# by256/icsg3d

Hardware: AMD Instinct MI355X
Metric: voxel-grids/s (fwd+bwd) for 32^3 U-Net+VAE at batch 32: value = U-Net train step (BASELINE configs[1]); DFC-VAE step (configs[2]) in secondary; both per batch in unet_plus_vae (higher is better)
Workload: dtype f32

## Files before the change

icsg3d_amd/csrc/common.h:

```cpp
#pragma once
#include <hip/hip_runtime.h>
#include <hip/hip_ext.h>
#include <atomic>
#include <cstdint>
#include <cstdio>
#include <string>
#include <vector>

namespace ics {

extern std::atomic<long long> g_kernel_launches;
struct LaunchTimer {
  virtual void next(hipEvent_t* start, hipEvent_t* stop) = 0;
  virtual ~LaunchTimer() = default;
};
extern thread_local LaunchTimer* tl_launch_timer;
template <typename... P, typename... A>
inline void ics_launch(void (*kernel)(P...), dim3 grid, dim3 block, size_t shmem, hipStream_t st, A&&... args) {
  static_assert(sizeof...(P) == sizeof...(A), "kernel argument count");
  if (tl_launch_timer != nullptr) {
    hipEvent_t e0 = nullptr, e1 = nullptr;
    tl_launch_timer->next(&e0, &e1);
    hipExtLaunchKernelGGL(kernel, grid, block, (std::uint32_t)shmem, st, e0, e1, 0u, static_cast<P>(args)...);
  } else {
    hipLaunchKernelGGL(kernel, grid, block, shmem, st, static_cast<P>(args)...);
  }
}
#define ICS_LAUNCH(...)                                      \
  do {                                                       \
    ::ics::g_kernel_launches.fetch_add(1, std::memory_order_relaxed); \
    ::ics::ics_launch(__VA_ARGS__);                          \
  } while (0)

void set_error(const std::string& msg);
#define ICS_HIP(expr)                                                                     \
  do {                                                                                    \
    hipError_t _e = (expr);                                                               \
    if (_e != hipSuccess) {                                                               \
      ::ics::set_error(std::string(#expr) + " -> " + hipGetErrorString(_e) + " @" +       \
                       __FILE__ + ":" + std::to_string(__LINE__));                        \
      return -1;                                                                          \
    }                                                                                     \
  } while (0)
#define ICS_CHECK(cond, msg)                                                              \
  do {                                                                                    \
    if (!(cond)) {                                                                        \
      ::ics::set_error(std::string(msg) + " (" #cond ") @" + __FILE__ + ":" +             \
                       std::to_string(__LINE__));                                         \
      return -1;                                                                          \
    }                                                                                     \
  } while (0)
#define ICS_TRY(expr)                                                                     \
  do {                                                                                    \
    if ((expr) != 0) return -1;                                                           \
  } while (0)

enum Act : int { ACT_NONE = 0, ACT_RELU = 1, ACT_LRELU = 2 };
constexpr float kLeaky = 0.3f;
constexpr float kBnEps = 1e-3f;
constexpr float kKEps = 1e-7f;
constexpr float kPoolTieTol = 1e-5f;

__device__ __forceinline__ float act_fwd(float v, int act) {
  if (act == ACT_RELU) return fmaxf(v, 0.f);
  if (act == ACT_LRELU) return v > 0.f ? v : kLeaky * v;
  return v;
}
__device__ __forceinline__ float act_grad(float v, int act) {
  if (act == ACT_RELU) return v > 0.f ? 1.f : 0.f;
  if (act == ACT_LRELU) return v > 0.f ? 1.f : kLeaky;
  return 1.f;
}

struct ConvSrc {
  const float* p;
  const float* scale;
  const float* shift;
  int C;
  int up;
  int act;
  int bcast;
};

enum ConvFlags : int {
  CF_NO_REUSE = 1,
  CF_NO_WGRAD3 = 2,
  CF_NO_WGRAD3S = 4,
  CF_NO_FWD_SPLITK = 8,
  CF_NO_THIN_N = 16,
  CF_NO_UPSPLIT = 32,
  CF_NO_THIN_C = 64,
  CF_NO_COND_FOLD = 128,
  CF_NO_WINO = 256,
  CF_NO_WINO_WGRAD = 512,
  CF_NO_WINO64 = 1024,
  CF_NO_UP3 = 2048,
  CF_NO_THIN1_2STAGE = 4096,
  CF_NO_FAST_BNBWD = 8192,
  CF_NO_FUSED_HEAD = 16384,
  CF_NO_BWD_FOLD = 32768,
  CF_UP3_BIG_ALWAYS = 65536,
  CF_NO_WINOG = 262144,
  CF_NO_HEAD_BNFUSE = 524288,
  CF_NO_UP3N = 1 << 21,
  CF_NO_DGRAD_BNFUSE = 1 << 22,
  CF_NO_POOL_PRESUM = 1 << 23,
  CF_NO_HEAD_LABELS = 1 << 24,
  CF_ZBATCH = 1 << 20,
};
int conv_flags_from_env();

struct ConvGeom {
  int B, S, lgS;
  int Cin, Cout;
  int taps;
  int Kpad, Npad;
  int flags = 0;
};

struct BwdStat {
  const float* s = nullptr;
  const float* mean = nullptr;
  const float* rstd = nullptr;
  const float* scale = nullptr;
  const float* shift = nullptr;
  float* partial = nullptr;
  int post_act = ACT_NONE;
  int ld = 0;
  const float* abc = nullptr;
  float* db_partial = nullptr;
  const float* pool_d = nullptr;
  int pool_ld = 0;
  const unsigned char* pool_mask = nullptr;
};

int launch_conv_fwd(hipStream_t st, const ConvGeom& g, const ConvSrc* src, int nsrc,
                    const float* wpacked, const float* bias, float* out, int ldo, int pre_act,
                    float* stat_partial, int* stat_rows_per_block, int accumulate = 0,
                    float* splitk_ws = nullptr, size_t splitk_ws_floats = 0, const BwdStat* bwd = nullptr,
                    int* bwd_blocks = nullptr);
size_t conv_fwd_workspace_floats(const ConvGeom& g, const ConvSrc* src, int nsrc);
bool conv_thin_c_ok(const ConvGeom& g, const ConvSrc& s0, int nsrc, int cin_log);
size_t conv_thin_c_wgrad_workspace_floats(const ConvGeom& g);
int launch_conv_wgrad_thin_c(hipStream_t st, const ConvGeom& g, const ConvSrc& s0, const float* dy, int ldy, float* dw,
                             int ldw, int row_pitch, float* ws, size_t ws_floats, int phase);
int launch_conv_fwd_thin_c(hipStream_t st, const ConvGeom& g, const ConvSrc& s0, int cin_log, int wstride,
                           const float* wp, const float* bias, float* out, int ldo, int pre_act, float* stat_partial,
                           int* rows_per_block, const float* pos_bias = nullptr);
int launch_conv_fwd_par(hipStream_t st, const ConvGeom& g_lowres, const ConvSrc& src, const float* wpar, float* out,
                        int ldo, const float* bias = nullptr, int pre_act = ACT_NONE, float* stat_partial = nullptr,
                        int* stat_blocks = nullptr);
int launch_pack_par(hipStream_t st, const float* w, int Cin_total, int Cout, int c_off, int Cu, float* dst, int Kpad,
                    int Npad);
int launch_pack_fwd_sub(hipStream_t st, const float* w, int taps, int Cin_total, int Cout, int c_off, int Csub,
                        float* dst, int Kpad, int Npad);
int launch_conv_wgrad(hipStream_t st, const ConvGeom& g, const ConvSrc* src, int nsrc,
                      const float* dy, int ldy, float* dw, int ldw, float* workspace,
                      size_t workspace_floats, int sub_rows = 0, int row_pitch = 0, int row_off = 0,
                      int phase = 0);
const char* conv_last_kernel_id();
void conv_set_last_kernel_id(const char* id);
int launch_pack_sub(hipStream_t st, const float* w, int taps, int Cin_total, int Cout, int c_off, int Csub,
                    int flip, float* dst, int Kpad, int Npad);
size_t conv_wgrad_workspace_floats(const ConvGeom& g, const ConvSrc* src, int nsrc);
int conv_fwd_rows_per_block(const ConvGeom& g);
int launch_conv_wgrad_ablate(hipStream_t st, const ConvGeom& g, const ConvSrc* src, const float* dy, int ldy,
                             float* workspace, int ablate);
int launch_conv_fwd_ablate(hipStream_t st, const ConvGeom& g, const ConvSrc* src, int nsrc, const float* wp,
                           float* out, int ldo, int ablate);
int launch_pack_fwd(hipStream_t st, const float* w, int K, int N, float* dst, int Kpad, int Npad,
                    int k_off, int n_off, int zero_first, int cin_log = 0, int cin_phys = 0);
void* pack_table_record_begin();
int pack_table_record_end(void* handle, std::vector<unsigned char>* bytes, int* njobs, unsigned* nblocks);
int launch_pack_table(hipStream_t st, const void* d_jobs, int njobs, unsigned nblocks);
int launch_materialize_input(hipStream_t st, const ConvSrc* src, int nsrc, int Cin, int CinG, int B, int S,
                             float* out);
int launch_pack_bwd(hipStream_t st, const float* w, int taps, int Cin, int Cout, float* dst,
                    int Kpad, int Npad, int cout_total, int co_off, int zero_first);

bool conv_wino_ok(const ConvGeom& g, const ConvSrc* src, int nsrc);
size_t conv_wino_weight_floats(int Cin, int Cout);
int launch_conv_fwd_wino(hipStream_t st, const ConvGeom& g, const ConvSrc& s0, const float* wt, const float* bias,
                         float* out, int ldo, int pre_act, float* stat_partial, int* rows_per_block, int accumulate,
                         int layout, const BwdStat* bwd = nullptr, int* bwd_blocks = nullptr);
int launch_pack_wino(hipStream_t st, const float* w, int Cin_total, int Cout, int c_off, int Csub, int bwd, float* dst,
                     int layout = 0);
int conv_wino_layout(const ConvGeom& g);
bool conv_wino64_ok(const ConvGeom& g, const ConvSrc* src, int nsrc);
int launch_conv_fwd_wino64(hipStream_t st, const ConvGeom& g, const ConvSrc& s0, const float* wt, const float* bias,
                           float* out, int ldo, int pre_act, float* stat_partial, int* rows_per_block, int accumulate,
                           const BwdStat* bwd = nullptr, int* bwd_blocks = nullptr);
bool conv_wino_wgrad_ok(const ConvGeom& g, const ConvSrc* src, int nsrc);
size_t conv_wino_wgrad_workspace_floats(const ConvGeom& g);
int launch_conv_wgrad_wino(hipStream_t st, const ConvGeom& g, const ConvSrc& s0, const float* dy, int ldy, float* dw,
// ... 26 lines not shown
```

icsg3d_amd/csrc/conv_igemm.hip:

```cpp
#include "common.h"

#ifndef ICS_GEMM_DEEP_FWD_MIN
#define ICS_GEMM_DEEP_FWD_MIN 1
#endif
#ifndef ICS_GEMM_DEEP_MIN
#define ICS_GEMM_DEEP_MIN 3
#endif
#ifndef ICS_GEMM_DEEP
#define ICS_GEMM_DEEP 1
#endif

#include <algorithm>
#include <type_traits>
#include <cstdlib>
#include <cstring>
#include <vector>

namespace ics {

typedef float f32x16 __attribute__((ext_vector_type(16)));
typedef float v4f __attribute__((ext_vector_type(4)));

#ifndef ICS_KLDA
#define ICS_KLDA 36
#endif
constexpr int kLDA = ICS_KLDA;

__device__ __forceinline__ int xcd_swizzle(int bid, int nblk) {
  const int xcd = bid & 7, q = nblk >> 3, r = nblk & 7;
  return (xcd < r ? xcd * (q + 1) : r * (q + 1) + (xcd - r) * q) + (bid >> 3);
}

static thread_local const char* g_last_kernel_id = "";
const char* conv_last_kernel_id() { return g_last_kernel_id; }
void conv_set_last_kernel_id(const char* id) { g_last_kernel_id = id; }
static const char* tf(bool b) { return b ? "true" : "false"; }

int conv_flags_from_env() {
  int f = 0;
  if (getenv("ICSG3D_NO_REUSE")) f |= CF_NO_REUSE;
  if (getenv("ICSG3D_NO_WGRAD3")) f |= CF_NO_WGRAD3;
  if (getenv("ICSG3D_NO_WGRAD3S")) f |= CF_NO_WGRAD3S;
  if (getenv("ICSG3D_NO_FWD_SPLITK")) f |= CF_NO_FWD_SPLITK;
  if (getenv("ICSG3D_NO_THIN_N")) f |= CF_NO_THIN_N;
  if (getenv("ICSG3D_NO_UPSPLIT")) f |= CF_NO_UPSPLIT;
  if (getenv("ICSG3D_NO_THIN_C")) f |= CF_NO_THIN_C;
  if (getenv("ICSG3D_NO_COND_FOLD")) f |= CF_NO_COND_FOLD;
  if (getenv("ICSG3D_NO_WINO")) f |= CF_NO_WINO;
  if (getenv("ICSG3D_NO_WINO_WGRAD")) f |= CF_NO_WINO_WGRAD;
  if (getenv("ICSG3D_NO_WINO64")) f |= CF_NO_WINO64;
  if (getenv("ICSG3D_NO_UP3")) f |= CF_NO_UP3;
  if (getenv("ICSG3D_NO_THIN1_2STAGE")) f |= CF_NO_THIN1_2STAGE;
  if (getenv("ICSG3D_NO_FAST_BNBWD")) f |= CF_NO_FAST_BNBWD;
  if (getenv("ICSG3D_NO_FUSED_HEAD")) f |= CF_NO_FUSED_HEAD;
  if (getenv("ICSG3D_NO_BWD_FOLD")) f |= CF_NO_BWD_FOLD;
  if (getenv("ICSG3D_NO_WINOG")) f |= CF_NO_WINOG;
  if (getenv("ICSG3D_NO_HEAD_BNFUSE")) f |= CF_NO_HEAD_BNFUSE;
  if (getenv("ICSG3D_NO_UP3N")) f |= CF_NO_UP3N;
  if (getenv("ICSG3D_NO_DGRAD_BNFUSE")) f |= CF_NO_DGRAD_BNFUSE;
  if (getenv("ICSG3D_NO_POOL_PRESUM")) f |= CF_NO_POOL_PRESUM;
  if (getenv("ICSG3D_NO_HEAD_LABELS")) f |= CF_NO_HEAD_LABELS;
  { const char* e = getenv("ICSG3D_UP3_BIG_MIN_WG"); if (e && *e && strtoul(e, nullptr, 10) <= 1) f |= CF_UP3_BIG_ALWAYS; }
  return f;
}
struct DevOnce {
  bool done[64] = {false};
  bool need(int* dev) {
    int d = 0;
    if (hipGetDevice(&d) != hipSuccess || d < 0 || d >= 64) { *dev = -1; return true; }
    *dev = d;
    return !done[d];
  }
  void mark(int dev) { if (dev >= 0) done[dev] = true; }
};

static int identity_affine(const float** ones, const float** zeros) {
  constexpr int kN = 16384;
  static float* buf[64] = {nullptr};
  int dev = 0;
  ICS_HIP(hipGetDevice(&dev));
  ICS_CHECK(dev >= 0 && dev < 64, "device index out of range");
  if (!buf[dev]) {
    float* p = nullptr;
    ICS_HIP(hipMalloc(&p, 2 * kN * sizeof(float)));
    std::vector<float> h(2 * kN, 0.f);
    for (int i = 0; i < kN; ++i) h[i] = 1.f;
    ICS_HIP(hipMemcpy(p, h.data(), 2 * kN * sizeof(float), hipMemcpyHostToDevice));
    buf[dev] = p;
  }
  *ones = buf[dev];
  *zeros = buf[dev] + kN;
  return 0;
}
static int fix_src(ConvSrc& s) {
  if (s.scale == nullptr) {
    ICS_CHECK(s.C <= 16384, "source wider than the identity-affine buffer");
    ICS_TRY(identity_affine(&s.scale, &s.shift));
    s.act = ACT_NONE;
  }
  return 0;
}

struct RowPos {
  int b, z, y, x;
};
__device__ __forceinline__ RowPos decode_row(int m, int S, int lg) {
  RowPos r;
  r.x = m & (S - 1);
  r.y = (m >> lg) & (S - 1);
  r.z = (m >> (2 * lg)) & (S - 1);
  r.b = m >> (3 * lg);
  return r;
}

// ... 10 lines not shown
}
__device__ __forceinline__ float act_apply(float v, float slope) {
  return fmaxf(v, v * slope);
}
template <bool NOACT>
__device__ __forceinline__ v4f affine_only_or_act4(v4f v, v4f sc, v4f sh, float slope);
__device__ __forceinline__ v4f affine_act4(v4f v, v4f sc, v4f sh, float slope) {
  v4f r;
  r.x = act_apply(fmaf(v.x, sc.x, sh.x), slope); r.y = act_apply(fmaf(v.y, sc.y, sh.y), slope);
  r.z = act_apply(fmaf(v.z, sc.z, sh.z), slope); r.w = act_apply(fmaf(v.w, sc.w, sh.w), slope);
  return r;
}
template <bool NOACT>
__device__ __forceinline__ v4f affine_only_or_act4(v4f v, v4f sc, v4f sh, float slope) {
  if (!NOACT) return affine_act4(v, sc, sh, slope);
  v4f r;
  r.x = fmaf(v.x, sc.x, sh.x); r.y = fmaf(v.y, sc.y, sh.y); r.z = fmaf(v.z, sc.z, sh.z); r.w = fmaf(v.w, sc.w, sh.w);
  return r;
}
__device__ __forceinline__ unsigned voxel_off(int b, int z, int y, int x, int S, int u, int C) {
  const int Ss = S >> u;
  return ((((unsigned)b * Ss + (z >> u)) * Ss + (y >> u)) * Ss + (x >> u)) * (unsigned)C;
}
__device__ __forceinline__ int clampi(int v, int hi) { return min(max(v, 0), hi); }

__device__ __forceinline__ ConvSrc pick_src(const ConvSrc& s0, const ConvSrc& s1, bool first) {
  ConvSrc s;
  s.p = first ? s0.p : s1.p;
  s.scale = first ? s0.scale : s1.scale;
  s.shift = first ? s0.shift : s1.shift;
  s.C = first ? s0.C : s1.C;
  s.up = first ? s0.up : s1.up;
  s.act = first ? s0.act : s1.act;
  s.bcast = first ? s0.bcast : s1.bcast;
  return s;
}

__device__ __forceinline__ float gather_scalar(const ConvSrc& s0, const ConvSrc& s1, int ci, int b,
                                               int z, int y, int x, int S) {
  const bool first = ci < s0.C;
  const ConvSrc s = pick_src(s0, s1, first);
  const int cl = first ? ci : ci - s0.C;
  float v;
  if (s.bcast > 0) {
    v = s.p[(size_t)b * s.bcast + (cl % s.bcast)];
  } else {
    v = s.p[src_voxel(s, b, z, y, x, S) + cl];
  }
  if (s.scale) v = act_fwd(fmaf(v, s.scale[cl], s.shift[cl]), s.act);
  return v;
}

template <int WM, int WN, int TM, int TN, bool VEC, int ABL = 0, bool AFF = true, bool UP = true, bool THIN = false,
          bool REUSE = false, bool PAR = false, bool NOACT = false, bool FOLD = false>
__global__ __launch_bounds__(256, FOLD ? 2 : ((REUSE && PAR) ? 3 : 1)) void conv_fwd_kernel(ConvGeom g, ConvSrc s0, ConvSrc s1,
                                                        const float* __restrict__ wp,
                                                        const float* __restrict__ bias,
                                                        float* __restrict__ out, int ldo, int pre_act,
                                                        float* __restrict__ stat_partial, int gridM,
                                                        int gridN, int accumulate, BwdStat bs) {
  constexpr int BM = WM * TM * 32, BN = WN * TN * 32;
  constexpr int B_FLOATS = 32 * BN;
  constexpr int RA = BM / 32;
  constexpr int RS = BM / 8;
  constexpr int NB = BN / 32;
  extern __shared__ __attribute__((aligned(16))) float smem[];
  const int A_FLOATS = (REUSE ? BM + (BM >> g.lgS) + 1 : BM) * kLDA;
  float* As = smem;
  constexpr int NABUF = 1;
  float* Bs = smem + NABUF * A_FLOATS;

  const int t = threadIdx.x, lane = t & 63, wave = t >> 6;
  const int wm = wave / WN, wn = wave % WN;
  const int li = lane & 31, lh = lane >> 5;
  const int sw = xcd_swizzle(blockIdx.x, gridM * gridN);
  const int mb = sw / gridN, nb = sw % gridN;
  const int S = g.S, lg = g.lgS;
  const int M = g.B << (3 * lg);
  const int n0 = nb * BN;
  const int nchunks = g.Kpad >> 5;
  const int cpt = (VEC && !THIN) ? (g.Cin >> 5) : 1;
  const int cls = PAR ? (int)blockIdx.y : 0;
  const int pz = cls >> 2, py = (cls >> 1) & 1, px = cls & 1;
  if (PAR) wp += (size_t)cls * g.Kpad * g.Npad;
  const bool zbatch = (g.flags & CF_ZBATCH) != 0;
  if (zbatch) {
    s0.p += (size_t)blockIdx.z * (size_t)M * (size_t)s0.C;
    wp += (size_t)blockIdx.z * (size_t)g.Kpad * (size_t)g.Npad;
    out += (size_t)blockIdx.z * (size_t)M * (size_t)ldo;
  }
  const int zsplit = zbatch ? 1 : (int)gridDim.z, zidx = zbatch ? 0 : (int)blockIdx.z;

  const int mrow_base = mb * BM + (VEC ? (t >> 3) : (t >> 5));
  const float slope0 = act_slope_of(s0.act), slope1 = act_slope_of(s1.act);
  const float pre_slope = act_slope_of(pre_act);

  unsigned rmask[RA];
  int rvh[RA];
  if (VEC) {
#pragma unroll
    for (int r = 0; r < RA; ++r) {
      const int m = mrow_base + 32 * r;
      const RowPos rp = decode_row(m, S, lg);
      unsigned mk = 0;
      if (m < M) {
        if (PAR) {
#pragma unroll
          for (int tp = 0; tp < 8; ++tp) {
            const int zz = rp.z + (tp >> 2) + pz - 1, yy = rp.y + ((tp >> 1) & 1) + py - 1, xx = rp.x + (tp & 1) + px - 1;
            const bool ok = (unsigned)zz < (unsigned)S && (unsigned)yy < (unsigned)S && (unsigned)xx < (unsigned)S;
            mk |= (ok ? 1u : 0u) << tp;
          }
#pragma unroll
// ... 118 lines not shown
#pragma unroll
      for (int r = 0; r < RA; ++r) {
        const unsigned mk = rmask[r];
        const bool inb = kvalid && ((mk >> (tap & 31)) & 1u);
        int idx = mrow_base + 32 * r + sdelta;
        if (UP) {
          const int ez = (dz + (int)((mk >> 29) & 1u)) >> 1;
          const int ey = (dy + (int)((mk >> 28) & 1u)) >> 1;
          const int ex = (dx + (int)((mk >> 27) & 1u)) >> 1;
          const int idx_up = rvh[r] + (ez * Sh + ey) * Sh + ex;
          idx = su ? idx_up : idx;
        }
        const unsigned off = inb ? (unsigned)idx * (unsigned)sC + cl : (unsigned)cl;
        if (ABL == 3) {
          ra4[r] = *reinterpret_cast<const v4f*>(sp + (((unsigned)(mrow_base + 32 * r) * sC + c * 32 + cl) & 0xffffffu));
          continue;
        }
        if (ABL == 8) {
          ra4[r] = *reinterpret_cast<const v4f*>(sp + ((unsigned)max(idx, 0) * (unsigned)sC + cl));
          continue;
        }
        if (ABL == 9) {
          const v4f vv = *reinterpret_cast<const v4f*>(sp + (((unsigned)(mrow_base + 32 * r) * sC + c * 32 + cl) & 0xffffffu));
          ra4[r] = inb ? vv : v4f{0.f, 0.f, 0.f, 0.f};
          continue;
        }
        v4f v = *reinterpret_cast<const v4f*>(sp + off);
        if (AFF && ABL != 4) v = affine_act4(v, sc, sh, slope);
        ra4[r] = inb ? v : v4f{0.f, 0.f, 0.f, 0.f};
      }
    } else {
      const int kf = (c << 5) + (t & 31);
      const int tap = kf / g.Cin, ci = kf - tap * g.Cin;
      const bool kvalid = tap < g.taps;
      int dz = 0, dy = 0, dx = 0;
      if (g.taps == 27) { dz = tap / 9 - 1; dy = (tap / 3) % 3 - 1; dx = tap % 3 - 1; }
#pragma unroll
      for (int r = 0; r < RS; ++r) {
        const int m = mrow_base + 8 * r;
        const RowPos rp = decode_row(m, S, lg);
        const int zz = rp.z + dz, yy = rp.y + dy, xx = rp.x + dx;
        const bool inb = kvalid && m < M && (unsigned)zz < (unsigned)S &&
                         (unsigned)yy < (unsigned)S && (unsigned)xx < (unsigned)S;
        ras[r] = inb ? gather_scalar(s0, s1, ci, rp.b, zz, yy, xx, S) : 0.f;
      }
    }
  };

  unsigned rowG0[RA], rowG1[RA];
  if (VEC) {
#pragma unroll
    for (int r = 0; r < RA; ++r) {
      const unsigned mc = (unsigned)min(mrow_base + 32 * r, M - 1);
      rowG0[r] = (mc * (unsigned)s0.C + (unsigned)(t & 7) * 4u) * 4u;
      rowG1[r] = (mc * (unsigned)s1.C + (unsigned)(t & 7) * 4u) * 4u;
    }
  }
  auto load_chunk_gemm = [&](int c) {
    load_b(c * 8);
    const int ci0 = c << 5;
    const bool first = ci0 < s0.C;
    const int cbase = first ? ci0 : ci0 - s0.C;
    const char* sp = reinterpret_cast<const char*>(first ? s0.p : s1.p) + (size_t)cbase * 4;
    const float slope = first ? slope0 : slope1;
    v4f sc = v4f{1.f, 1.f, 1.f, 1.f}, sh = v4f{0.f, 0.f, 0.f, 0.f};
    if (AFF) {
      sc = *reinterpret_cast<const v4f*>((first ? s0.scale : s1.scale) + cbase + (t & 7) * 4);
      sh = *reinterpret_cast<const v4f*>((first ? s0.shift : s1.shift) + cbase + (t & 7) * 4);
    }
#pragma unroll
    for (int r = 0; r < RA; ++r) {
      v4f v = *reinterpret_cast<const v4f*>(sp + (first ? rowG0[r] : rowG1[r]));
      if (AFF) v = affine_only_or_act4<NOACT>(v, sc, sh, slope);
      ra4[r] = v;
    }
  };
  auto store_a_chunk = [&]() {
    float* A = As;
    if (VEC) {
#pragma unroll
      for (int r = 0; r < RA; ++r)
        *reinterpret_cast<v4f*>(A + ((t >> 3) + 32 * r) * kLDA + (t & 7) * 4) = ra4[r];
    } else {
#pragma unroll
      for (int r = 0; r < RS; ++r) A[((t >> 5) + 8 * r) * kLDA + (t & 31)] = ras[r];
    }
  };

  f32x16 acc[TM][TN];
#pragma unroll
  for (int i = 0; i < TM; ++i)
#pragma unroll
    for (int j = 0; j < TN; ++j)
#pragma unroll
      for (int r = 0; r < 16; ++r) acc[i][j][r] = 0.f;
  if (accumulate && !PAR && zsplit == 1) {
#pragma unroll
    for (int j = 0; j < TN; ++j) {
      const int n = n0 + wn * TN * 32 + j * 32 + li;
#pragma unroll
      for (int i = 0; i < TM; ++i)
#pragma unroll
        for (int r = 0; r < 16; ++r) {
          const int m = mb * BM + wm * TM * 32 + 4 * lh + i * 32 + (r & 3) + 8 * (r >> 2);
          if (m < M && n < g.Cout) acc[i][j][r] = out[(size_t)m * ldo + n];
        }
    }
  }

  auto compute_at = [&](const float* Abase, int arow_stride_rows, int bbuf) {
    const float* Bw = Bs + bbuf * B_FLOATS + (lh * BN + wn * TN * 32 + li) * 4;
#pragma unroll
    for (int g8 = 0; g8 < 4; ++g8) {
      float4 a[TM], b[TN];
#pragma unroll
      for (int i = 0; i < TM; ++i)
// ... 73 lines not shown
    store_b(par);
    __syncthreads();
    for (int G = G0; G + 1 < G1; ++G) {
      int ngzy = gzy, ncc = cc + 1;
      if (ncc == cpt) { ncc = 0; ++ngzy; }
      load_a_group(ngzy, ncc);
#pragma unroll
      for (int i = 0; i < NDX; ++i) {
        load_b(i + 1 < NDX ? b_rows(gzy, cc, i + 1) : b_rows(ngzy, ncc, 0));
        compute_reuse(0, par, dx_first + i);
        par ^= 1;
        store_b(par);
        __syncthreads();
      }
      store_a_group(0);
      __syncthreads();
      gzy = ngzy; cc = ncc;
    }
    {
#pragma unroll
      for (int i = 0; i + 1 < NDX; ++i) {
        load_b(b_rows(gzy, cc, i + 1));
        compute_reuse(0, par, dx_first + i);
        par ^= 1;
        store_b(par);
        __syncthreads();
      }
      compute_reuse(0, par, dx_first + NDX - 1);
      __syncthreads();
    }
    }
  } else {
  int cb = 0, ce = nchunks;
  if (zsplit > 1) {
    const int per = (nchunks + zsplit - 1) / zsplit;
    cb = zidx * per;
    ce = min(nchunks, cb + per);
  }
  const bool gemm = VEC && !THIN && !PAR && !UP && ABL == 0 && g.taps == 1;
  if (cb < ce && gemm) {
    auto compute_g = [&](int buf) { compute_at(As + (wm * TM * 32 + li) * kLDA + lh * 4, 32, buf); };
    load_chunk_gemm(cb);
    store_b(cb & 1);
    store_a_chunk();
    __syncthreads();
#if ICS_GEMM_DEEP
    if (!AFF && TM * TN >= ICS_GEMM_DEEP_FWD_MIN) {
      v4f raA[RA], rbA[NB], raB[RA], rbB[NB];
      auto load_set = [&](int c, v4f (&xa)[RA], v4f (&xb)[NB]) {
        const char* wrow = reinterpret_cast<const char*>(wp) + (size_t)(c * 8) * (size_t)g.Npad * 16;
#pragma unroll
        for (int r = 0; r < NB; ++r) xb[r] = *reinterpret_cast<const v4f*>(wrow + bofs[r]);
        const int ci0 = c << 5;
        const bool first = ci0 < s0.C;
        const char* sp = reinterpret_cast<const char*>(first ? s0.p : s1.p) + (size_t)(first ? ci0 : ci0 - s0.C) * 4;
#pragma unroll
        for (int r = 0; r < RA; ++r) xa[r] = *reinterpret_cast<const v4f*>(sp + (first ? rowG0[r] : rowG1[r]));
      };
      auto store_set = [&](int buf, const v4f (&xa)[RA], const v4f (&xb)[NB]) {
        float* Bw = Bs + buf * B_FLOATS;
#pragma unroll
        for (int r = 0; r < NB; ++r) *reinterpret_cast<v4f*>(Bw + (t + 256 * r) * 4) = xb[r];
        __syncthreads();
#pragma unroll
        for (int r = 0; r < RA; ++r) *reinterpret_cast<v4f*>(As + ((t >> 3) + 32 * r) * kLDA + (t & 7) * 4) = xa[r];
        __syncthreads();
      };
      const int lastc = ce - 1;
      if (cb + 1 < ce) load_set(cb + 1, raA, rbA);
      int c = cb;
      for (; c + 2 < ce; c += 2) {
        load_set(c + 2, raB, rbB);
        compute_g(c & 1);
        store_set((c + 1) & 1, raA, rbA);
        load_set(c + 3 < ce ? c + 3 : lastc, raA, rbA);
        compute_g((c + 1) & 1);
        store_set(c & 1, raB, rbB);
      }
      if (c + 1 < ce) {
        compute_g(c & 1);
        store_set((c + 1) & 1, raA, rbA);
      }
      compute_g((ce - 1) & 1);
      __syncthreads();
    } else
#endif
    {
    for (int c = cb; c + 1 < ce; ++c) {
      load_chunk_gemm(c + 1);
      compute_g(c & 1);
      store_b((c + 1) & 1);
      __syncthreads();
      store_a_chunk();
      __syncthreads();
    }
    compute_g((ce - 1) & 1);
    __syncthreads();
    }
  } else if (cb < ce) {
  load_chunk(cb);
  store_b(cb & 1);
  store_a_chunk();
  __syncthreads();

  auto compute = [&](int buf) {
    compute_at(As + (wm * TM * 32 + li) * kLDA + lh * 4, 32, buf);
  };
  auto compute_regs_only = [&]() {
// ... 111 lines not shown
  }
  if (stat_partial == nullptr) return;

  float* red = smem;
  float* bmean = smem + WM * BN;
  const int nvalid_rows = min(BM, M - mb * BM);
#pragma unroll
  for (int j = 0; j < TN; ++j) {
    float cs = colsum[j];
    cs += __shfl_xor(cs, 32);
    if (lh == 0) red[wm * BN + wn * TN * 32 + j * 32 + li] = cs;
  }
  __syncthreads();
  if (t < BN) {
    float s = 0.f;
#pragma unroll
    for (int w = 0; w < WM; ++w) s += red[w * BN + t];
    bmean[t] = s / (float)nvalid_rows;
  }
  __syncthreads();
#pragma unroll
  for (int j = 0; j < TN; ++j) {
    const float mu = bmean[wn * TN * 32 + j * 32 + li];
    float q = 0.f;
#pragma unroll
    for (int i = 0; i < TM; ++i)
#pragma unroll
      for (int r = 0; r < 16; ++r) {
        const int m = mrow0 + i * 32 + (r & 3) + 8 * (r >> 2);
        const float d = acc[i][j][r] - mu;
        q += (m < M) ? d * d : 0.f;
      }
    q += __shfl_xor(q, 32);
    colsum[j] = q;
  }
  __syncthreads();
#pragma unroll
  for (int j = 0; j < TN; ++j)
    if (lh == 0) red[wm * BN + wn * TN * 32 + j * 32 + li] = colsum[j];
  __syncthreads();
  if (t < BN) {
    float q = 0.f;
#pragma unroll
    for (int w = 0; w < WM; ++w) q += red[w * BN + t];
    const size_t nstat = (size_t)(PAR ? 8 : 1) * gridM;
    float* sp = stat_partial + (size_t)(n0 + t) * nstat + (size_t)(cls * gridM + mb);
    sp[0] = (float)nvalid_rows;
    sp[(size_t)g.Npad * nstat] = bmean[t];
    sp[(size_t)2 * g.Npad * nstat] = q;
  }
}

template <int WM, int WN, int TM, int TN, bool VEC, int ABL = 0, bool AFF = true, bool UP = true, bool THIN = false,
          bool REUSE = false, bool PAR = false, bool NOACT = false, bool FOLD = false>
static int launch_fwd_cfg(hipStream_t st, const ConvGeom& g, const ConvSrc& s0, const ConvSrc& s1,
                          const float* wp, const float* bias, float* out, int ldo, int pre_act,
                          float* stat_partial, int* rows_per_block, int accumulate = 0, int ksplit = 1,
                          const BwdStat* bwd = nullptr) {
  constexpr int BM = WM * TM * 32, BN = WN * TN * 32;
  const int M = g.B << (3 * g.lgS);
  const int gridM = (M + BM - 1) / BM, gridN = g.Npad / BN;
  const int arows = REUSE ? BM + (BM >> g.lgS) + 1 : BM;
  const size_t lds = (size_t)(arows * kLDA + 2 * 32 * BN) * sizeof(float);
  auto kern = conv_fwd_kernel<WM, WN, TM, TN, VEC, ABL, AFF, UP, THIN, REUSE, PAR, NOACT, FOLD>;
  static DevOnce attr;
  int dev;
  if (attr.need(&dev)) {
    const size_t lds_max = (size_t)((REUSE ? BM + BM / 4 + 1 : BM) * kLDA + 2 * 32 * BN) * sizeof(float);
    ICS_HIP(hipFuncSetAttribute(reinterpret_cast<const void*>(kern),
                                hipFuncAttributeMaxDynamicSharedMemorySize, (int)lds_max));
    attr.mark(dev);
  }
  if (rows_per_block) *rows_per_block = BM;
  static const std::string id = std::string("conv_fwd_kernel<") + std::to_string(WM) + ", " + std::to_string(WN) + ", " +
                                std::to_string(TM) + ", " + std::to_string(TN) + ", " + tf(VEC) + ", " +
                                std::to_string(ABL) + ", " + tf(AFF) + ", " + tf(UP) + ", " + tf(THIN) + ", " +
                                tf(REUSE) + ", " + tf(PAR) + ", " + tf(NOACT) + ", " + tf(FOLD) + ">";
  g_last_kernel_id = id.c_str();
  BwdStat bs_arg;
  if (FOLD) bs_arg = *bwd;
  ICS_LAUNCH(kern, dim3(gridM * gridN, PAR ? 8 : 1, ksplit), dim3(256), lds, st, g, s0, s1, wp, bias, out, ldo,
                     pre_act, stat_partial, gridM, gridN, accumulate, bs_arg);
  ICS_HIP(hipGetLastError());
  return 0;
}

static void pick_fwd_tile(const ConvGeom& g, int* bm, int* bn) {
  const int M = g.B << (3 * g.lgS);
  int BN = (g.Npad % 128 == 0) ? 128 : (g.Npad % 96 == 0) ? 96 : (g.Npad % 64 == 0) ? 64 : 32;
  int BM = 128;
  if (g.Npad % 64 == 0 && (long)((M + 127) / 128) * (g.Npad / BN) < 384) {
    BM = 64;
    BN = 64;
  }
  *bm = BM;
  *bn = BN;
}

static bool fwd_is_vec(const ConvGeom& g, const ConvSrc& s0, const ConvSrc& s1) {
  return (g.Cin % 32 == 0) && (s0.C % 32 == 0) && s0.bcast == 0 && s1.bcast == 0;
}
static bool conv_is_thin(const ConvGeom& g, const ConvSrc& s0, int nsrc) {
  return nsrc == 1 && s0.bcast == 0 && s0.C == g.Cin && (g.Cin == 4 || g.Cin == 8 || g.Cin == 16);
}


int launch_gemm_zbatch(hipStream_t st, int nz, int M, int K, int N, const float* A, const float* Wp, float* out, int flags) {
  ICS_CHECK(nz >= 1 && nz <= 65535 && M >= 1 && K % 32 == 0 && N % 64 == 0, "z-batched GEMM: K % 32, N % 64 required");
  ICS_CHECK((size_t)M * (size_t)std::max(K, N) < ((size_t)1 << 30), "z-batched GEMM: matrix too large for 32-bit offsets");
  const ConvGeom g{M, 1, 0, K, N, 1, K, N, flags | CF_ZBATCH};
  const ConvSrc s0{A, nullptr, nullptr, K, 0, ACT_NONE, 0}, s1{};
#ifndef ICS_ZB_BIG
#define ICS_ZB_BIG 1
#endif
  if (ICS_ZB_BIG && M % 128 == 0 && N % 128 == 0 && (long)(M / 128) * (N / 128) * nz >= 512)
    return launch_fwd_cfg<2, 2, 2, 2, true, 0, false, false, false, false, false, true, false>(
        st, g, s0, s1, Wp, nullptr, out, N, ACT_NONE, nullptr, nullptr, 0, nz);
  return launch_fwd_cfg<2, 2, 1, 1, true, 0, false, false, false, false, false, true, false>(
      st, g, s0, s1, Wp, nullptr, out, N, ACT_NONE, nullptr, nullptr, 0, nz);
}

int conv_fwd_rows_per_block(const ConvGeom& g) {
  int bm, bn;
  pick_fwd_tile(g, &bm, &bn);
  if (g.taps == 27 && g.Cout <= 4 && g.Cin % 4 == 0 && g.Cin >= 4 && g.Cin <= 64) {
    bm = std::min(bm, g.Cin <= 16 ? 256 : 64);
  }
  return bm;
}

#ifndef ICS_THINC_UNROLL
#define ICS_THINC_UNROLL 3
#endif
template <int CIN, int COUT>
__global__ __launch_bounds__(256) void conv_thin_c_fwd_kernel(ConvGeom g, const float* __restrict__ x, int wstride,
                                                               const float* __restrict__ wp,
                                                               const float* __restrict__ bias,
                                                               float* __restrict__ out, int ldo, int pre_act,
                                                               float* __restrict__ stat_partial,
                                                               const float* __restrict__ pos_bias) {
  constexpr int LPV = COUT / 4;
  constexpr int GPB = 256 / LPV;
  constexpr int VPB = 4 * GPB;
  constexpr int C4 = CIN >= 4 ? CIN / 4 : 1;
  extern __shared__ __attribute__((aligned(16))) float smem[];
  float* w = smem;
  const int t = threadIdx.x;
  const int S = g.S, lg = g.lgS;
  const int M = g.B << (3 * lg);
// ... 734 lines not shown
  if (ks > 1 && (size_t)ks * ((size_t)g.B << (3 * g.lgS)) * g.Npad > ws_floats) ks = 1;
  if (bwd_blocks) *bwd_blocks = 0;
  if (ks <= 1) {
    const bool fold = bwd != nullptr && bwd->partial != nullptr && !thin_n_ok(g, src[0], nsrc) &&
                      fwd_is_vec(g, s0, s1) && !conv_is_thin(g, s0, nsrc) && s0.scale == nullptr && !s0.up &&
                      (nsrc < 2 || (s1.scale == nullptr && !s1.up)) && bias == nullptr && stat_partial == nullptr &&
                      !accumulate;
    int rpb = 0;
    ICS_TRY(launch_conv_fwd_inner(st, g, src, nsrc, wp, bias, out, ldo, pre_act, stat_partial, &rpb, accumulate, 1,
                                  fold ? bwd : nullptr, ws, ws_floats));
    if (rows_per_block) *rows_per_block = rpb;
    if (fold && bwd_blocks) *bwd_blocks = (int)((((size_t)g.B << (3 * g.lgS)) + rpb - 1) / rpb);
    return 0;
  }
  const int M = g.B << (3 * g.lgS);
  ICS_CHECK((size_t)ks * M * g.Npad <= ws_floats, "forward split-K workspace too small");
  ICS_TRY(launch_conv_fwd_inner(st, g, src, nsrc, wp, nullptr, ws, g.Npad, ACT_NONE, nullptr, nullptr, 0, ks));
  ICS_LAUNCH(splitk_finish_kernel, dim3((M + 63) / 64, (g.Npad + 63) / 64), dim3(256), 0, st, ws, ks, M, g.Cout,
                     g.Npad, bias, act_slope_of(pre_act), out, ldo, accumulate, stat_partial);
  ICS_HIP(hipGetLastError());
  if (rows_per_block) *rows_per_block = 64;
  return 0;
}

static int launch_conv_fwd_inner(hipStream_t st, const ConvGeom& g, const ConvSrc* src, int nsrc,
                                 const float* wp, const float* bias, float* out, int ldo, int pre_act,
                                 float* stat_partial, int* rows_per_block, int accumulate, int ksplit,
                                 const BwdStat* bwd, float* ws, size_t ws_floats) {
  if (ksplit == 1 && thin_n_ok(g, src[0], nsrc))
    return launch_thin_n_fwd(st, g, src[0], wp, bias, out, ldo, pre_act, stat_partial, rows_per_block, accumulate, ws,
                             ws_floats);
  if (ksplit == 1 && !accumulate && bwd == nullptr && conv_thin_c_ok(g, src[0], nsrc, g.Cin) && ldo % 4 == 0)
    return launch_conv_fwd_thin_c(st, g, src[0], g.Cin, g.Cin, wp, bias, out, ldo, pre_act, stat_partial,
                                  rows_per_block);
  ConvSrc s0 = src[0], s1 = src[nsrc > 1 ? 1 : 0];
  if (nsrc == 1) s1.C = 0;
  const bool aff = s0.scale != nullptr || (nsrc > 1 && s1.scale != nullptr);
  const bool up = s0.up || (nsrc > 1 && s1.up);
  const int variant = up ? 2 : (aff ? 1 : 0);
  const bool noact = aff && (s0.scale == nullptr || s0.act == ACT_NONE) &&
                     (nsrc < 2 || s1.scale == nullptr || s1.act == ACT_NONE);
  ICS_TRY(fix_src(s0));
  ICS_TRY(fix_src(s1));
  bool vec = fwd_is_vec(g, s0, s1);
  const bool thin = conv_is_thin(g, s0, nsrc);
  ICS_CHECK(((size_t)g.B << (3 * g.lgS)) * (size_t)std::max(s0.C, s1.C) * 4 <= 0xffffffffull,
            "conv source larger than 4 GiB");
  const bool no_reuse = (g.flags & CF_NO_REUSE) != 0;
  const bool fold = bwd != nullptr && bwd->partial != nullptr && ksplit == 1 && vec && !thin && variant == 0 &&
                    bias == nullptr && stat_partial == nullptr && !accumulate;
  int bm, bn;
  pick_fwd_tile(g, &bm, &bn);
#define ICS_FWD_ARGS st, g, s0, s1, wp, bias, out, ldo, pre_act, stat_partial, rows_per_block, accumulate, ksplit, bwd
#define ICS_FWD(WM, WN, TM, TN)                                                                 \
  do {                                                                                          \
    if (thin) return launch_fwd_cfg<WM, WN, TM, TN, true, 0, true, true, true>(ICS_FWD_ARGS);   \
    if (!vec) return launch_fwd_cfg<WM, WN, TM, TN, false, 0, true, true>(ICS_FWD_ARGS);        \
    if (g.taps == 27 && g.S >= 4 && g.S <= (WM) * (TM) * 32 && !no_reuse) {                      \
      if (variant == 0 && fold)                                                                 \
        return launch_fwd_cfg<WM, WN, TM, TN, true, 0, false, false, false, true, false, false, true>(ICS_FWD_ARGS); \
      if (variant == 0) return launch_fwd_cfg<WM, WN, TM, TN, true, 0, false, false, false, true>(ICS_FWD_ARGS); \
      if (variant == 1 && noact)                                                                \
        return launch_fwd_cfg<WM, WN, TM, TN, true, 0, true, false, false, true, false, true>(ICS_FWD_ARGS);     \
      if (variant == 1) return launch_fwd_cfg<WM, WN, TM, TN, true, 0, true, false, false, true>(ICS_FWD_ARGS);  \
      return launch_fwd_cfg<WM, WN, TM, TN, true, 0, true, true, false, true>(ICS_FWD_ARGS);    \
    }                                                                                           \
    if (variant == 0 && fold)                                                                   \
      return launch_fwd_cfg<WM, WN, TM, TN, true, 0, false, false, false, false, false, false, true>(ICS_FWD_ARGS); \
    if (variant == 0) return launch_fwd_cfg<WM, WN, TM, TN, true, 0, false, false>(ICS_FWD_ARGS); \
    if (variant == 1) return launch_fwd_cfg<WM, WN, TM, TN, true, 0, true, false>(ICS_FWD_ARGS);  \
    return launch_fwd_cfg<WM, WN, TM, TN, true, 0, true, true>(ICS_FWD_ARGS);                   \
  } while (0)
  if (bm == 64) { ICS_FWD(2, 2, 1, 1); }
  if (bn == 128) { ICS_FWD(2, 2, 2, 2); }
  if (bn == 96) { ICS_FWD(4, 1, 1, 3); }
  if (bn == 64) { ICS_FWD(2, 2, 2, 1); }
  ICS_FWD(4, 1, 1, 1);
#undef ICS_FWD_ARGS
#undef ICS_FWD
}

static void pick_par_tile(const ConvGeom& g, int* bm, int* bn) {
  pick_fwd_tile(g, bm, bn);
  if (*bm == 64 && g.Npad % 128 == 0 && (long)(((g.B << (3 * g.lgS)) + 127) / 128) * (g.Npad / 128) * 8 >= 384) {
    *bm = 128; *bn = 128;
  }
}
int launch_conv_fwd_par(hipStream_t st, const ConvGeom& g, const ConvSrc& src, const float* wp, float* out,
                        int ldo, const float* bias, int pre_act, float* stat_partial, int* stat_blocks) {
  ConvSrc s0 = src, s1 = src;
  s1.C = 0;
  ICS_CHECK(g.taps == 8 && g.Cin % 32 == 0 && s0.C == g.Cin && !s0.up && !s0.bcast && g.Kpad == 8 * g.Cin,
            "parity-class conv needs a direct 32k-channel source");
  ICS_TRY(fix_src(s0));
  ICS_TRY(fix_src(s1));
  int bm, bn;
  pick_par_tile(g, &bm, &bn);
  int rpb = 0;
#define ICS_PAR_ARGS st, g, s0, s1, wp, bias, out, ldo, pre_act, stat_partial, &rpb
  int rc;
  const bool no_reuse = (g.flags & CF_NO_REUSE) != 0;
  const bool reuse = !no_reuse && g.S >= 4 && g.S <= bm;
  const bool noact = src.scale != nullptr && src.act == ACT_NONE;
#define ICS_PAR(WM, WN, TM, TN)                                                                              \
  (reuse ? (noact ? launch_fwd_cfg<WM, WN, TM, TN, true, 0, true, false, false, true, true, true>(ICS_PAR_ARGS) \
                  : launch_fwd_cfg<WM, WN, TM, TN, true, 0, true, false, false, true, true>(ICS_PAR_ARGS))   \
// ... 58 lines not shown
  const size_t total = (size_t)8 * Kpad * Npad;
  ICS_LAUNCH(pack_par_kernel, dim3((unsigned)((total + 255) / 256)), dim3(256), 0, st, w, Cin_total, Cout,
                     c_off, Cu, dst, Kpad, Npad);
  ICS_HIP(hipGetLastError());
  return 0;
}
__device__ __forceinline__ float pack_fwd_sub_value(size_t i, const float* __restrict__ w, int taps, int Cin_total,
                                                    int Cout, int c_off, int Csub, int Npad) {
  const int tq = i & 3;
  const size_t rest = i >> 2;
  const int n = rest % Npad;
  const int k = (int)(rest / Npad) * 4 + tq;
  const int tap = k / Csub, c = k - tap * Csub;
  return (tap < taps && n < Cout) ? w[((size_t)tap * Cin_total + c_off + c) * Cout + n] : 0.f;
}
__global__ void pack_fwd_sub_kernel(const float* __restrict__ w, int taps, int Cin_total, int Cout, int c_off,
                                    int Csub, float* __restrict__ dst, int Kpad, int Npad) {
  const size_t i = (size_t)blockIdx.x * blockDim.x + threadIdx.x;
  if (i >= (size_t)Kpad * Npad) return;
  dst[i] = pack_fwd_sub_value(i, w, taps, Cin_total, Cout, c_off, Csub, Npad);
}
int launch_pack_fwd_sub(hipStream_t st, const float* w, int taps, int Cin_total, int Cout, int c_off, int Csub,
                        float* dst, int Kpad, int Npad) {
  if (g_pack_rec) { g_pack_rec->push_back(PackJob{3, w, dst, {taps, Cin_total, Cout, c_off, Csub, Npad, 0, 0, 0}, (unsigned long long)Kpad * Npad, 0}); return 0; }
  const size_t total = (size_t)Kpad * Npad;
  ICS_LAUNCH(pack_fwd_sub_kernel, dim3((unsigned)((total + 255) / 256)), dim3(256), 0, st, w, taps,
                     Cin_total, Cout, c_off, Csub, dst, Kpad, Npad);
  ICS_HIP(hipGetLastError());
  return 0;
}

int launch_conv_fwd_ablate(hipStream_t st, const ConvGeom& g, const ConvSrc* src, int nsrc, const float* wp,
                           float* out, int ldo, int ablate) {
  ConvSrc s0 = src[0], s1 = src[nsrc > 1 ? 1 : 0];
  if (nsrc == 1) s1.C = 0;
  ICS_TRY(fix_src(s0));
  ICS_TRY(fix_src(s1));
  ICS_CHECK(fwd_is_vec(g, s0, s1) && g.Npad % 128 == 0, "ablation bench needs the vector 128x128 configuration");
#define ICS_ABL_ARGS st, g, s0, s1, wp, nullptr, out, ldo, 0, nullptr, nullptr
  if (ablate == 1) return launch_fwd_cfg<2, 2, 2, 2, true, 1, true, false>(ICS_ABL_ARGS);
  if (ablate == 2) return launch_fwd_cfg<2, 2, 2, 2, true, 2, true, false>(ICS_ABL_ARGS);
  if (ablate == 3) return launch_fwd_cfg<2, 2, 2, 2, true, 3, true, false>(ICS_ABL_ARGS);
  if (ablate == 4) return launch_fwd_cfg<2, 2, 2, 2, true, 4, true, false>(ICS_ABL_ARGS);
  if (ablate == 8) return launch_fwd_cfg<2, 2, 2, 2, true, 8, false, false>(ICS_ABL_ARGS);
  if (ablate == 9) return launch_fwd_cfg<2, 2, 2, 2, true, 9, false, false>(ICS_ABL_ARGS);
  if (ablate == 5) return launch_fwd_cfg<2, 2, 2, 2, true, 0, true, false>(ICS_ABL_ARGS);
  if (ablate == 6) return launch_fwd_cfg<2, 2, 2, 2, true, 0, true, true>(ICS_ABL_ARGS);
  return launch_fwd_cfg<2, 2, 2, 2, true, 0, false, false>(ICS_ABL_ARGS);
#undef ICS_ABL_ARGS
}


template <int WM, int WN, int TM, int TN, bool VEC, bool DYVEC, bool AFF = true, bool UP = true, bool THIN = false,
          int ABL = 0>
__global__ __launch_bounds__(256) void conv_wgrad_kernel(ConvGeom g, ConvSrc s0, ConvSrc s1,
                                                          const float* __restrict__ dy, int ldy,
                                                          int n_load,
                                                          float* __restrict__ ws, int ktiles,
                                                          int ntiles, int rows_per_split) {
  constexpr int KT = WM * TM * 32, NT = WN * TN * 32;
  constexpr int A_FLOATS = 32 * KT, D_FLOATS = 32 * NT;
  constexpr int AF4 = KT / 4, ATOT = 32 * AF4, APASS = ATOT / 256;
  constexpr int DF4 = NT / 4, DTOT = 32 * DF4, DPASS = DTOT / 256;
  static_assert(ATOT % 256 == 0 && DTOT % 256 == 0, "tile loads must divide evenly over 256 threads");
  extern __shared__ __attribute__((aligned(16))) float smem[];
  float* As = smem;
  float* Ds = smem + 2 * A_FLOATS;

  const int t = threadIdx.x, lane = t & 63, wave = t >> 6;
  const int wm = wave / WN, wn = wave % WN;
  const int li = lane & 31, lh = lane >> 5;
  const int S = g.S, lg = g.lgS;
  const int M = g.B << (3 * lg);
  const int K = g.taps * g.Cin;

  int bid = blockIdx.x;
  const int nt_i = bid % ntiles; bid /= ntiles;
  const int kt_i = bid % ktiles; bid /= ktiles;
  const int split = bid;
  const int n0 = nt_i * NT;
  const int m_begin = split * rows_per_split;
  const int m_end = min(M, m_begin + rows_per_split);
  const int nchunks = (m_end - m_begin + 31) >> 5;

  const int k0 = kt_i * KT;
  int tdz = 0, tdy = 0, tdx = 0, sdelta = 0, xbad = -1, ybad = -1, zbad = -1;
  bool kvalid = false;
  const float* sp = s0.p;
  int sC = s0.C, su = 0, cl0 = 0;
  float slope = 1.f;
  v4f sc = v4f{1.f, 1.f, 1.f, 1.f}, sh = v4f{0.f, 0.f, 0.f, 0.f};
  if (VEC) {
    const int kf = k0 + (t % AF4) * 4;
    const int tap = kf / g.Cin, ci = kf - tap * g.Cin;
    kvalid = kf < K;
    if (g.taps == 27 && kvalid) { tdz = tap / 9 - 1; tdy = (tap / 3) % 3 - 1; tdx = tap % 3 - 1; }
    sdelta = (tdz * S + tdy) * S + tdx;
    xbad = tdx < 0 ? 0 : (tdx > 0 ? S - 1 : -1);
    ybad = tdy < 0 ? 0 : (tdy > 0 ? S - 1 : -1);
    zbad = tdz < 0 ? 0 : (tdz > 0 ? S - 1 : -1);
    const bool first = ci < s0.C;
    const ConvSrc sv = pick_src(s0, s1, first);
    sp = sv.p; sC = sv.C; su = sv.up;
    cl0 = kvalid ? (first ? ci : ci - s0.C) : 0;
    slope = act_slope_of(sv.act);
    if (AFF) {
      sc = *reinterpret_cast<const v4f*>(sv.scale + cl0);
      sh = *reinterpret_cast<const v4f*>(sv.shift + cl0);
    }
  }
  int s_tap = 0, s_ci = 0; bool s_kvalid = false; int sdz = 0, sdy = 0, sdx = 0;
  if (!VEC) {
// ... 11 lines not shown
    if (VEC) {
      const int Sh = S >> 1;
#pragma unroll
      for (int p = 0; p < APASS; ++p) {
        const int m = mbase + (t + 256 * p) / AF4;
        const int x = m & (S - 1), y = (m >> lg) & (S - 1), z = (m >> (2 * lg)) & (S - 1);
        const bool inb = kvalid && m < m_end && x != xbad && y != ybad && z != zbad;
        int idx = m + sdelta;
        if (UP) {
          const int b = m >> (3 * lg);
          const int idx_up = ((b * Sh + ((z + tdz) >> 1)) * Sh + ((y + tdy) >> 1)) * Sh + ((x + tdx) >> 1);
          idx = su ? idx_up : idx;
        }
        const unsigned off = inb ? (unsigned)idx * (unsigned)sC + cl0 : (unsigned)cl0;
        v4f v = *reinterpret_cast<const v4f*>(sp + off);
        if (AFF) v = affine_act4(v, sc, sh, slope);
        ra[p] = inb ? v : v4f{0.f, 0.f, 0.f, 0.f};
      }
    } else {
#pragma unroll
      for (int p = 0; p < 4; ++p) {
        const int m = mbase + (t >> 5) + 8 * p;
        float v = 0.f;
        if (s_kvalid && m < m_end) {
          const RowPos r = decode_row(m, S, lg);
          const int zz = r.z + sdz, yy = r.y + sdy, xx = r.x + sdx;
          if ((unsigned)zz < (unsigned)S && (unsigned)yy < (unsigned)S && (unsigned)xx < (unsigned)S)
            v = gather_scalar(s0, s1, s_ci, r.b, zz, yy, xx, S);
        }
        ras[p] = v;
      }
    }
#pragma unroll
    for (int p = 0; p < DPASS; ++p) {
      const int idx = t + 256 * p;
      const int m = mbase + idx / DF4;
      const int n = n0 + (idx % DF4) * 4;
      const float* q = dy + (size_t)min(m, M - 1) * ldy;
      v4f v;
      if (DYVEC) {
        v = *reinterpret_cast<const v4f*>(q + min(n, n_load - 4));
        if (!(m < m_end && n < n_load)) v = v4f{0.f, 0.f, 0.f, 0.f};
      } else {
        v.x = q[min(n + 0, n_load - 1)]; v.y = q[min(n + 1, n_load - 1)];
        v.z = q[min(n + 2, n_load - 1)]; v.w = q[min(n + 3, n_load - 1)];
        const bool rowok = m < m_end;
        v.x = (rowok && n + 0 < n_load) ? v.x : 0.f; v.y = (rowok && n + 1 < n_load) ? v.y : 0.f;
        v.z = (rowok && n + 2 < n_load) ? v.z : 0.f; v.w = (rowok && n + 3 < n_load) ? v.w : 0.f;
      }
      rd[p] = v;
    }
  };
  const bool gemm = VEC && DYVEC && !UP && !THIN && ABL == 0 && g.taps == 1 && (M & 31) == 0 &&
                    (rows_per_split & 31) == 0 && n0 + NT <= n_load;
  const bool noact_g = slope == 1.f;
  unsigned aoffg[VEC ? APASS : 1], doffg[DPASS];
  if (VEC) {
#pragma unroll
    for (int p = 0; p < APASS; ++p) aoffg[p] = (unsigned)(((t + 256 * p) / AF4) * sC + cl0) * 4u;
  }
#pragma unroll
  for (int p = 0; p < DPASS; ++p) {
    const int idx = t + 256 * p;
    doffg[p] = (unsigned)((idx / DF4) * ldy + n0 + (idx % DF4) * 4) * 4u;
  }
  auto load_chunk_gemm = [&](int c, auto noact_tag) {
    constexpr bool NA = decltype(noact_tag)::value;
    const int mbase = m_begin + (c << 5);
    const char* abase = reinterpret_cast<const char*>(sp) + (size_t)mbase * (size_t)sC * 4;
    const char* dbase = reinterpret_cast<const char*>(dy) + (size_t)mbase * (size_t)ldy * 4;
    if (VEC) {
#pragma unroll
      for (int p = 0; p < APASS; ++p) {
        v4f v = *reinterpret_cast<const v4f*>(abase + aoffg[p]);
        if (AFF) v = affine_only_or_act4<NA>(v, sc, sh, slope);
        ra[p] = v;
      }
    }
#pragma unroll
    for (int p = 0; p < DPASS; ++p) rd[p] = *reinterpret_cast<const v4f*>(dbase + doffg[p]);
  };
  auto store_chunk = [&](int buf) {
    float* A = As + buf * A_FLOATS;
    float* D = Ds + buf * D_FLOATS;
    if (VEC) {
#pragma unroll
      for (int p = 0; p < APASS; ++p) {
        const int idx = t + 256 * p;
        *reinterpret_cast<v4f*>(A + (idx / AF4) * KT + (idx % AF4) * 4) = ra[p];
      }
    } else {
#pragma unroll
      for (int p = 0; p < 4; ++p) A[((t >> 5) + 8 * p) * KT + (t & 31)] = ras[p];
    }
#pragma unroll
    for (int p = 0; p < DPASS; ++p) {
      const int idx = t + 256 * p;
      *reinterpret_cast<v4f*>(D + (idx / DF4) * NT + (idx % DF4) * 4) = rd[p];
    }
  };

  f32x16 acc[TM][TN];
#pragma unroll
  for (int i = 0; i < TM; ++i)
#pragma unroll
    for (int j = 0; j < TN; ++j)
#pragma unroll
      for (int r = 0; r < 16; ++r) acc[i][j][r] = 0.f;

  if (nchunks > 0) {
    if (gemm && noact_g) load_chunk_gemm(0, std::true_type{});
    else if (gemm) load_chunk_gemm(0, std::false_type{});
    else load_chunk(0);
    store_chunk(0);
  }
  __syncthreads();
  constexpr bool SPLIT_M = (TM != 3), SPLIT_N = (TN != 3);
  auto compute = [&](int buf) {
    const float* A = As + buf * A_FLOATS + lh * KT + wm * TM * 32 + (SPLIT_M ? TM * li : li);
    const float* D = Ds + buf * D_FLOATS + lh * NT + wn * TN * 32 + (SPLIT_N ? TN * li : li);
#pragma unroll
    for (int s = 0; s < 16; ++s) {
      float a[TM], b[TN];
      if (SPLIT_M && TM == 2) {
        const float2 q = *reinterpret_cast<const float2*>(A + s * 2 * KT);
        a[0] = q.x; a[1 % TM] = q.y;
      } else if (SPLIT_M && TM == 4) {
        const float4 q = *reinterpret_cast<const float4*>(A + s * 2 * KT);
        a[0] = q.x; a[1 % TM] = q.y; a[2 % TM] = q.z; a[3 % TM] = q.w;
      } else {
#pragma unroll
        for (int i = 0; i < TM; ++i) a[i] = A[s * 2 * KT + i * 32];
      }
      if (SPLIT_N && TN == 2) {
        const float2 q = *reinterpret_cast<const float2*>(D + s * 2 * NT);
        b[0] = q.x; b[1 % TN] = q.y;
      } else if (SPLIT_N && TN == 4) {
        const float4 q = *reinterpret_cast<const float4*>(D + s * 2 * NT);
        b[0] = q.x; b[1 % TN] = q.y; b[2 % TN] = q.z; b[3 % TN] = q.w;
      } else {
#pragma unroll
        for (int j = 0; j < TN; ++j) b[j] = D[s * 2 * NT + j * 32];
      }
#pragma unroll
      for (int i = 0; i < TM; ++i)
#pragma unroll
        for (int j = 0; j < TN; ++j)
          acc[i][j] = __builtin_amdgcn_mfma_f32_32x32x2f32(a[i], b[j], acc[i][j], 0, 0, 0);
    }
  };
#if ICS_GEMM_DEEP
  if (gemm && VEC && TM * TN >= ICS_GEMM_DEEP_MIN) {
    v4f raA[APASS], rdA[DPASS], raB[APASS], rdB[DPASS];
    auto loadS = [&](int c, v4f (&xa)[APASS], v4f (&xd)[DPASS]) {
      const int mbase = m_begin + (c << 5);
      const char* abase = reinterpret_cast<const char*>(sp) + (size_t)mbase * (size_t)sC * 4;
      const char* dbase = reinterpret_cast<const char*>(dy) + (size_t)mbase * (size_t)ldy * 4;
#pragma unroll
      for (int p = 0; p < APASS; ++p) xa[p] = *reinterpret_cast<const v4f*>(abase + aoffg[p]);
#pragma unroll
      for (int p = 0; p < DPASS; ++p) xd[p] = *reinterpret_cast<const v4f*>(dbase + doffg[p]);
    };
    auto storeS = [&](int buf, const v4f (&xa)[APASS], const v4f (&xd)[DPASS]) {
      float* A = As + buf * A_FLOATS;
      float* D = Ds + buf * D_FLOATS;
#pragma unroll
      for (int p = 0; p < APASS; ++p) {
        const int idx = t + 256 * p;
        v4f v = xa[p];
        if (AFF) v = noact_g ? affine_only_or_act4<true>(v, sc, sh, slope) : affine_only_or_act4<false>(v, sc, sh, slope);
        *reinterpret_cast<v4f*>(A + (idx / AF4) * KT + (idx % AF4) * 4) = v;
      }
#pragma unroll
      for (int p = 0; p < DPASS; ++p) {
        const int idx = t + 256 * p;
        *reinterpret_cast<v4f*>(D + (idx / DF4) * NT + (idx % DF4) * 4) = xd[p];
      }
    };
    const int last = nchunks - 1;
    if (nchunks > 1) loadS(1, raA, rdA);
    int c = 0;
    for (; c + 2 < nchunks; c += 2) {
      loadS(c + 2, raB, rdB);
      compute(c & 1);
      storeS((c + 1) & 1, raA, rdA);
      __syncthreads();
      loadS(c + 3 < nchunks ? c + 3 : last, raA, rdA);
      compute((c + 1) & 1);
      storeS(c & 1, raB, rdB);
      __syncthreads();
    }
    if (c + 1 < nchunks) {
      compute(c & 1);
      storeS((c + 1) & 1, raA, rdA);
      __syncthreads();
    }
  } else
#endif
  if (gemm) {
    for (int c = 0; c + 1 < nchunks; ++c) {
      if (noact_g) load_chunk_gemm(c + 1, std::true_type{}); else load_chunk_gemm(c + 1, std::false_type{});
      compute(c & 1);
      store_chunk((c + 1) & 1);
      __syncthreads();
    }
  } else {
  for (int c = 0; c + 1 < nchunks; ++c) {
    if (ABL == 0 || ABL == 2) load_chunk(ABL == 2 ? 1 : c + 1);
    compute(c & 1);
    if (ABL == 0 || ABL == 2) store_chunk((c + 1) & 1);
// ... 453 lines not shown
    }
  };
  for (int c = 0; c + 1 < nchunks; ++c) {
    load_chunk(c + 1);
    compute(c & 1);
    store_chunk((c + 1) & 1);
    __syncthreads();
  }
  if (nchunks > 0) compute((nchunks - 1) & 1);

  float* wsp = ws + (size_t)split * K * g.Cout;
  const int n = n0 + 32 * wave + li;
#pragma unroll
  for (int dxi = 0; dxi < 3; ++dxi)
#pragma unroll
    for (int j = 0; j < 2; ++j)
#pragma unroll
      for (int r = 0; r < 16; ++r) {
        const int row = (r & 3) + 8 * (r >> 2) + 4 * lh;
        const int k = (gzy * 3 + dxi) * g.Cin + c0 + 2 * row + j;
        wsp[(size_t)k * g.Cout + n] = acc[dxi][j][r];
      }
}

static bool wgrad3_ok(const ConvGeom& g, const ConvSrc& s0, int nsrc, const ConvSrc& s1) {
  if ((g.flags & CF_NO_WGRAD3) || g.taps != 27 || g.S > 64 || g.S < 2 || g.Cin % 64 != 0 || g.Cout % 128 != 0) return false;
  if (s0.bcast || (nsrc > 1 && s1.bcast)) return false;
  if (nsrc > 1 && (s0.C % 64 != 0)) return false;
  return true;
}
struct Wgrad3Plan { int cgroups, ntiles, ksplit, rows_per_split; };
static Wgrad3Plan plan_wgrad3(const ConvGeom& g) {
  Wgrad3Plan p;
  const long M = (long)g.B << (3 * g.lgS);
  p.cgroups = g.Cin / 64;
  p.ntiles = g.Cout / 128;
  const int want = pick_ksplit(9L * p.cgroups * p.ntiles, M, g.lgS > 5 ? 512 : 768, 2);
  p.rows_per_split = (int)(((M + want - 1) / want + 31) / 32 * 32);
  p.ksplit = (int)((M + p.rows_per_split - 1) / p.rows_per_split);
  return p;
}


size_t conv_wgrad_workspace_floats(const ConvGeom& g, const ConvSrc* src, int nsrc) {
  if (thin_n_ok(g, src[0], nsrc)) return (size_t)thin_n_wgrad_splits(g) * g.taps * g.Cin * g.Cout;
  ConvSrc s0 = src[0], s1 = src[nsrc > 1 ? 1 : 0];
  WgradPlan p = plan_wgrad(g, s0, nsrc, s1);
  int ks = p.ksplit;
  if (wgrad3_ok(g, s0, nsrc, s1)) ks = std::max(ks, plan_wgrad3(g).ksplit);
  return (size_t)ks * g.taps * g.Cin * g.Cout;
}

template <int WM, int WN, int TM, int TN, bool VEC, bool DYVEC, bool AFF = true, bool UP = true, bool THIN = false,
          int ABL = 0>
static int launch_wgrad_cfg(hipStream_t st, const ConvGeom& g, const ConvSrc& s0, const ConvSrc& s1,
                            const float* dy, int ldy, int n_load, float* ws, const WgradPlan& p) {
  constexpr int KT = WM * TM * 32, NT = WN * TN * 32;
  const size_t lds = (size_t)2 * 32 * (KT + NT) * sizeof(float);
  auto kern = conv_wgrad_kernel<WM, WN, TM, TN, VEC, DYVEC, AFF, UP, THIN, ABL>;
  static DevOnce attr;
  int dev;
  if (attr.need(&dev)) {
    ICS_HIP(hipFuncSetAttribute(reinterpret_cast<const void*>(kern),
                                hipFuncAttributeMaxDynamicSharedMemorySize, (int)lds));
    attr.mark(dev);
  }
  static const std::string id = std::string("conv_wgrad_kernel<") + std::to_string(WM) + ", " + std::to_string(WN) +
                                ", " + std::to_string(TM) + ", " + std::to_string(TN) + ", " + tf(VEC) + ", " +
                                tf(DYVEC) + ", " + tf(AFF) + ", " + tf(UP) + ", " + tf(THIN) + ", " +
                                std::to_string(ABL) + ">";
  g_last_kernel_id = id.c_str();
  ICS_LAUNCH(kern, dim3(p.ktiles * p.ntiles * p.ksplit), dim3(256), lds, st, g, s0, s1, dy,
                     ldy, n_load, ws, p.ktiles, p.ntiles, p.rows_per_split);
  ICS_HIP(hipGetLastError());
  return 0;
}

int launch_conv_wgrad_ablate(hipStream_t st, const ConvGeom& g, const ConvSrc* src, const float* dy, int ldy,
                             float* workspace, int ablate) {
  ConvSrc s0 = src[0], s1 = src[0];
  s1.C = 0;
  ICS_TRY(fix_src(s0));
  ICS_TRY(fix_src(s1));
  WgradPlan p = plan_wgrad(g, s0, 1, s1);
  ICS_CHECK(p.vec && p.kt == 128 && p.nt == 128, "ablation bench needs the vector 128x128 configuration");
  if (ablate == 1) return launch_wgrad_cfg<2, 2, 2, 2, true, true, false, false, false, 1>(st, g, s0, s1, dy, ldy, g.Cout, workspace, p);
  return launch_wgrad_cfg<2, 2, 2, 2, true, true, false, false, false, 2>(st, g, s0, s1, dy, ldy, g.Cout, workspace, p);
}

int launch_conv_wgrad(hipStream_t st, const ConvGeom& g, const ConvSrc* src, int nsrc,
                      const float* dy, int ldy, float* dw, int ldw, float* workspace,
                      size_t workspace_floats, int sub_rows, int row_pitch, int row_off, int phase) {
  if (thin_n_ok(g, src[0], nsrc)) {
    const int ns = thin_n_wgrad_splits(g);
    const size_t n_el = (size_t)g.taps * g.Cin * g.Cout;
    ICS_CHECK((size_t)ns * n_el <= workspace_floats, "wgrad workspace too small");
    const int M = g.B << (3 * g.lgS);
    const int rows = (M + ns - 1) / ns;
    const int K = 27 * g.Cin;
    const bool aff = src[0].scale != nullptr;
    if (thin1_wgrad_ok(g, src[0])) {
      const int nb = thin1_wgrad_blocks(g);
      if (phase != 2) {
#define ICS_T1W(CKV)                                                                                                 \
  do {                                                                                                               \
    if (aff) ICS_LAUNCH((thin1_wgrad_kernel<CKV, true>), dim3(nb), dim3(256), 0, st, g, src[0], dy, ldy, workspace); \
    else ICS_LAUNCH((thin1_wgrad_kernel<CKV, false>), dim3(nb), dim3(256), 0, st, g, src[0], dy, ldy, workspace);    \
  } while (0)
        switch (g.Cin / 16) { case 1: ICS_T1W(1); break; case 2: ICS_T1W(2); break; case 3: ICS_T1W(3); break; default: ICS_T1W(4); break; }
#undef ICS_T1W
        ICS_HIP(hipGetLastError());
        g_last_kernel_id = "thin1_wgrad_kernel";
      }
      if (phase != 1) ICS_TRY(launch_reduce_splits(st, workspace, 4 * nb, n_el, g.Cout, dw, ldw, sub_rows, row_pitch, row_off));
      return 0;
    }
    if (phase != 2) {
#define ICS_TNW(NOUT, AFFV, KPT, NAME)                                                                         \
  do {                                                                                                         \
    g_last_kernel_id = NAME;                                                                                   \
    ICS_LAUNCH((conv_thin_n_wgrad_kernel<NOUT, AFFV, KPT>), dim3((M + rows - 1) / rows), dim3(256), 0,  \
                       st, g, src[0], dy, ldy, workspace, rows);                                               \
  } while (0)
#define ICS_TNW_K(NOUT, AFFV, TAG)                                                                  \
  do {                                                                                              \
    if (K <= 512) ICS_TNW(NOUT, AFFV, 2, "conv_thin_n_wgrad_kernel<" TAG ", 2>");                   \
// ... 39 lines not shown
      const bool noact = aff && (src[0].scale == nullptr || src[0].act == ACT_NONE) &&
                         (nsrc < 2 || src[1].scale == nullptr || src[1].act == ACT_NONE);
      const int ar = 32 + (g.lgS == 6 ? 1 : (32 >> g.lgS)) + 1;
      const size_t lds3 = (size_t)(2 * (ar * 64 + 32 * 128) + 128) * sizeof(float);
#define ICS_W3S(AFFV, NOACTV, LGV)                                                                              \
  do {                                                                                                          \
    g_last_kernel_id = "conv_wgrad3s_kernel<" #AFFV ", " #NOACTV ", " #LGV ">";                                 \
    ICS_LAUNCH((conv_wgrad3s_kernel<AFFV, NOACTV, LGV>), grid, dim3(256), lds3, st, g, s0, s1, dy, ldy,  \
                       workspace, q.cgroups, q.ntiles, q.rows_per_split);                                       \
  } while (0)
#define ICS_W3S_L(AFFV, NOACTV)                                                       \
  do {                                                                                \
    if (g.lgS == 4) ICS_W3S(AFFV, NOACTV, 4);                                         \
    else if (g.lgS == 5) ICS_W3S(AFFV, NOACTV, 5);                                    \
    else ICS_W3S(AFFV, NOACTV, 6);                                                    \
  } while (0)
      if (!aff) ICS_W3S_L(false, false);
      else if (noact) ICS_W3S_L(true, true);
      else ICS_W3S_L(true, false);
#undef ICS_W3S_L
#undef ICS_W3S
      ICS_HIP(hipGetLastError());
    } else if (phase != 2) {
#define ICS_W3(AFFV, UPV, HALOV)                                                                                 \
  do {                                                                                                           \
    g_last_kernel_id = "conv_wgrad3_kernel<" #AFFV ", " #UPV ", " #HALOV ">";                                    \
    ICS_LAUNCH((conv_wgrad3_kernel<AFFV, UPV, HALOV>), grid, dim3(256), lds, st, g, s0, s1, dy, ldy,      \
                       n_load, workspace, q.cgroups, q.ntiles, q.rows_per_split);                                \
  } while (0)
      if (g.lgS > 5) {
        if (up) ICS_W3(true, true, true); else if (aff) ICS_W3(true, false, true); else ICS_W3(false, false, true);
      } else {
        if (up) ICS_W3(true, true, false); else if (aff) ICS_W3(true, false, false); else ICS_W3(false, false, false);
      }
#undef ICS_W3
      ICS_HIP(hipGetLastError());
    }
    if (phase != 1) {
      ICS_TRY(launch_reduce_splits(st, workspace, q.ksplit, n_elems, g.Cout, dw, ldw, sub_rows, row_pitch, row_off));
    }
    return 0;
  }
  ICS_CHECK((size_t)p.ksplit * n_elems <= workspace_floats, "wgrad workspace too small");
  if (phase != 2) {
#define ICS_WG_ARGS st, g, s0, s1, dy, ldy, n_load, workspace, p
#define ICS_WG(WM, WN, TM, TN, DV)                                                                 \
  do {                                                                                             \
    if (p.thin) ICS_TRY((launch_wgrad_cfg<WM, WN, TM, TN, true, DV, true, true, true>(ICS_WG_ARGS)));  \
    else if (!p.vec) ICS_TRY((launch_wgrad_cfg<WM, WN, TM, TN, false, DV, true, true>(ICS_WG_ARGS)));   \
    else if (up) ICS_TRY((launch_wgrad_cfg<WM, WN, TM, TN, true, DV, true, true>(ICS_WG_ARGS)));   \
    else if (aff) ICS_TRY((launch_wgrad_cfg<WM, WN, TM, TN, true, DV, true, false>(ICS_WG_ARGS))); \
    else ICS_TRY((launch_wgrad_cfg<WM, WN, TM, TN, true, DV, false, false>(ICS_WG_ARGS)));         \
  } while (0)
  if (!dy_vec) {
    if (p.kt == 128) ICS_WG(4, 1, 1, 1, false);
    else if (p.kt == 64) ICS_WG(2, 2, 1, 1, false);
    else ICS_WG(1, 4, 1, 1, false);
  } else if (p.kt == 128) {
    if (p.nt == 128) ICS_WG(2, 2, 2, 2, true);
    else if (p.nt == 96) ICS_WG(4, 1, 1, 3, true);
    else if (p.nt == 64) ICS_WG(4, 1, 1, 2, true);
    else ICS_WG(4, 1, 1, 1, true);
  } else if (p.kt == 64) {
    if (p.nt == 128) ICS_WG(2, 2, 1, 2, true);
    else ICS_WG(2, 2, 1, 1, true);
  } else {
    ICS_WG(1, 4, 1, 1, true);
  }
#undef ICS_WG_ARGS
#undef ICS_WG
  }
  if (phase != 1) {
    ICS_TRY(launch_reduce_splits(st, workspace, p.ksplit, n_elems, g.Cout, dw, ldw, sub_rows, row_pitch, row_off));
  }
  return 0;
}

__device__ __forceinline__ bool pack_fwd_value(size_t i, const float* __restrict__ w, int K, int N, int Npad, int k_off,
                                               int n_off, int cin_log, int cin_phys, float* v) {
  const int tq = i & 3;
  const size_t rest = i >> 2;
  const int n = rest % Npad;
  const int k = (int)(rest / Npad) * 4 + tq;
  int ks = k - k_off;
  const int ns = n - n_off;
  bool ok = ks >= 0 && ks < K && ns >= 0 && ns < N;
  if (ok && cin_phys > 0) {
    const int tap = ks / cin_phys, ci = ks - tap * cin_phys;
    ok = ci < cin_log;
    ks = tap * cin_log + ci;
  }
  *v = ok ? w[(size_t)ks * N + ns] : 0.f;
  return ok;
}
__global__ void pack_fwd_kernel(const float* __restrict__ w, int K, int N, float* __restrict__ dst,
                                int Kpad, int Npad, int k_off, int n_off, int zero_first, int cin_log,
                                int cin_phys) {
  const size_t i = (size_t)blockIdx.x * blockDim.x + threadIdx.x;
  const size_t total = (size_t)Kpad * Npad;
  if (i >= total) return;
  float v;
  if (pack_fwd_value(i, w, K, N, Npad, k_off, n_off, cin_log, cin_phys, &v) || zero_first) dst[i] = v;
}

__global__ void materialize_input_kernel(ConvSrc s0, ConvSrc s1, int Cin, int CinG, int S, int lg, size_t total,
                                         float* __restrict__ out) {
  const size_t i = (size_t)blockIdx.x * blockDim.x + threadIdx.x;
// ... 335 lines not shown
```

icsg3d_amd/csrc/elementwise.h:

```cpp
#pragma once
#include "common.h"

#include <rccl/rccl.h>

namespace ics {

struct BnParams {
  const float* gamma;
  const float* beta;
  float* moving_mean;
  float* moving_var;
  float* mean;
  float* rstd;
  float* scale;
  float* shift;
  float* xs = nullptr;
};

struct BnSyncEmu {
  int rank, nranks;
  double* fwd;
  double* bwd;
  int cmax, cap;
  int call;
// ... 65 lines not shown
                      const BwdStat* bs, int Npad, int* blocks, const float* c1c2 = nullptr, float* db_partial = nullptr);
int launch_xhat_affine(hipStream_t st, const float* mean, const float* rstd, int C, float* xs);
int launch_head_bnfuse(hipStream_t st, const float* Q, const float* dzsum, const float* wsoft, const float* wsig,
                       const float* gamma, const float* beta, double n, int ncls, float* dwsoft, float* dwsig, float* c1c2,
                       float* dgamma, float* dbeta, const BnSync* sync = nullptr);
bool conv_bnfuse_ok(int S, int Cin, int N);
size_t conv_bnfuse_partial_floats(int B, int S, int C);
int launch_conv_bnfuse(hipStream_t st, const float* dy, int B, int S, int Cin, int CinTot, int N, const float* db_partial,
                       int db_nblk, const float* W, float* G, const float* gamma, const float* beta, const float* mean,
                       const float* rstd, const float* scale, float* abc, float* c1c2, float* dgamma, float* dbeta,
                       float* ws_partial, size_t ws_partial_floats, double* ws_R, double* sums_out = nullptr);
bool pool_presum_ok(int C, int ldg);
int pool_presum_blocks(size_t pooled_rows);
int launch_pool_presum(hipStream_t st, const float* g, int ldg, const unsigned char* mask, const float* ssum, size_t pooled_rows,
                       int C, const float* mean, const float* rstd, float* pre, size_t pre_floats, int* blocks);
size_t pool_bnfuse_partial_doubles(size_t pooled_rows, int C);
int launch_pool_bnfuse(hipStream_t st, const float* g, int ldg, const unsigned char* mask, const float* ssum, size_t pooled_rows,
                       int C, double cnt, const double* sums_conv, const float* mean, const float* rstd, const float* scale,
                       float* abc, float* c1c2, float* dgamma, float* dbeta, double* ws_partial, size_t ws_partial_doubles);
int launch_head_fused(hipStream_t st, const float* x, int ldx, const float* scale, const float* shift, const float* wsoft_k,
                      const float* wsig_k, const float* bsoft, const float* bsig, float* z, const unsigned char* labels,
                      size_t M, int mode, int want_grad, float wsoft, double* partial, int partial_blocks, float* metrics,
                      int* nblk_out = nullptr, float* dz_colsum = nullptr, double* keep = nullptr,
                      float thresh = 0.f, unsigned char* species = nullptr, unsigned char* mask = nullptr,
                      const float* cw = nullptr);
int launch_head(hipStream_t st, float* z, int ldz, int ncls, const unsigned char* labels, size_t M,
                int mode, int want_grad, float wsoft, double* partial, int partial_blocks,
                float* metrics, int* nblk_out = nullptr, float* dz_colsum = nullptr, double* keep = nullptr,
                const float* cw = nullptr);
int launch_head_metrics(hipStream_t st, const double* partial, int nblk, double M, float* metrics, double* sums,
                        int phase, double* keep = nullptr);
int launch_adam(hipStream_t st, float* p, const float* g, float* m, float* v, size_t n, float lr_t,
                float gscale);
int launch_bn_apply(hipStream_t st, const float* s, const float* scale, const float* shift, int act,
                    size_t n, int C, float* out);
int launch_sqdiff(hipStream_t st, const float* a, const float* b, int B, size_t per_sample,
                  int blocks_per_sample, double* partial, float* grad, float coef, int accumulate);
int launch_sampling(hipStream_t st, const float* mulv, int ld, int latent, const float* eps,
                    const float* cond, int ncond, int B, float* z, float* zc);
int launch_vae_loss(hipStream_t st, const float* mulv, int ld, int latent, int B, const double* mse_partial,
                    int n_mse, double n_elems, const double* pm_partial, const PmSums& pmc, float alpha, float beta,
                    float* metrics, double* sums = nullptr, int phase = 0);
int launch_vae_dz(hipStream_t st, const float* mulv, int ld, int latent, int B, const float* eps,
                  const float* dzc, int ldzc, float beta, float* dmulv);
int launch_cond_bias_table(hipStream_t st, const float* w, const float* bias, const float* cond, int C, int ncond,
                           int Cin_tot, int Cout, int B, float* T);
size_t cond_wgrad_workspace_doubles(int B, int Cout);
int launch_cond_wgrad(hipStream_t st, const float* dy, int B, int S, int Cout, const float* cond, int C0, int nfold,
                      int ncond, int Cin_tot, float* dw, double* ws, size_t ws_doubles);
int launch_relu_bwd(hipStream_t st, const float* a, float* g, size_t n);
int launch_colsum_small(hipStream_t st, const float* a, int rows, int cols, int ld, float* out);
int launch_axpy(hipStream_t st, float* y, const float* x, size_t n, float a);
int launch_pool27(hipStream_t st, const float* dy, int B, int S, int N, float* out, int ldo);
int launch_permute_up_dw(hipStream_t st, const float* tmp, int Cu, int N, int Cin, int c_off, float* dw);

}
```

icsg3d_amd/csrc/elementwise.hip:

```cpp
#include "common.h"
#include "elementwise.h"

namespace ics {

__device__ __forceinline__ double wave_sum_d(double v) {
#pragma unroll
  for (int o = 32; o > 0; o >>= 1) v += __shfl_xor(v, o);
  return v;
}
__device__ __forceinline__ float wave_sum_f(float v) {
#pragma unroll
  for (int o = 32; o > 0; o >>= 1) v += __shfl_xor(v, o);
  return v;
}
__device__ __forceinline__ float wave_max_f(float v) {
#pragma unroll
  for (int o = 32; o > 0; o >>= 1) v = fmaxf(v, __shfl_xor(v, o));
  return v;
}
__device__ __forceinline__ double block_sum_d(double v, double* sh ) {
  v = wave_sum_d(v);
  __syncthreads();
  if ((threadIdx.x & 63) == 0) sh[threadIdx.x >> 6] = v;
  __syncthreads();
// ... 1763 lines not shown
  size_t vl = i / N4;
  const int c = vl % Sh; size_t r = vl / Sh;
  const int bq = r % Sh; r /= Sh;
  const int a = r % Sh;
  const int b = (int)(r / Sh);
  pf4 o[27];
#pragma unroll
  for (int k = 0; k < 27; ++k) o[k] = pf4{0.f, 0.f, 0.f, 0.f};
#pragma unroll
  for (int sz = 0; sz < 4; ++sz) {
    const int z = 2 * a - 1 + sz;
    if ((unsigned)z >= (unsigned)S) continue;
    pf4 lx[4][3];
#pragma unroll
    for (int sy = 0; sy < 4; ++sy) {
      const int y = 2 * bq - 1 + sy;
      pf4 v[4];
#pragma unroll
      for (int sx = 0; sx < 4; ++sx) {
        const int x = 2 * c - 1 + sx;
        const bool ok = (unsigned)y < (unsigned)S && (unsigned)x < (unsigned)S;
        v[sx] = ok ? *reinterpret_cast<const pf4*>(dy + ((((size_t)b * S + z) * S + y) * S + x) * N + n) : pf4{0.f, 0.f, 0.f, 0.f};
      }
      lx[sy][2] = v[0] + v[1];
      lx[sy][1] = v[1] + v[2];
      lx[sy][0] = v[2] + v[3];
    }
    pf4 P[3][3];
#pragma unroll
    for (int dx = 0; dx < 3; ++dx) {
      P[2][dx] = lx[0][dx] + lx[1][dx];
      P[1][dx] = lx[1][dx] + lx[2][dx];
      P[0][dx] = lx[2][dx] + lx[3][dx];
    }
#pragma unroll
    for (int dyi = 0; dyi < 3; ++dyi)
#pragma unroll
      for (int dx = 0; dx < 3; ++dx) {
        if (sz <= 1) o[2 * 9 + dyi * 3 + dx] += P[dyi][dx];
        if (sz >= 1 && sz <= 2) o[1 * 9 + dyi * 3 + dx] += P[dyi][dx];
        if (sz >= 2) o[0 * 9 + dyi * 3 + dx] += P[dyi][dx];
      }
  }
#pragma unroll
  for (int k = 0; k < 27; ++k) *reinterpret_cast<pf4*>(out + vl * ldo + (size_t)k * N + n) = o[k];
}
int launch_pool27(hipStream_t st, const float* dy, int B, int S, int N, float* out, int ldo) {
  ICS_CHECK(N % 4 == 0 && ldo % 4 == 0, "pool27: channel counts must be multiples of 4");
  const size_t total = (size_t)B * (S / 2) * (S / 2) * (S / 2) * (N / 4);
  ICS_LAUNCH(pool27_kernel, dim3((unsigned)((total + 255) / 256)), dim3(256), 0, st, dy, B, S, N, total, out, ldo);
  ICS_HIP(hipGetLastError());
  return 0;
}
__global__ void permute_up_dw_kernel(const float* __restrict__ tmp, int Cu, int N, int Cin, int c_off,
                                     size_t total, float* __restrict__ dw) {
  const size_t i = (size_t)blockIdx.x * blockDim.x + threadIdx.x;
  if (i >= total) return;
  const int n = (int)(i % N);
  size_t r = i / N;
  const int c = (int)(r % Cu);
  const int tap = (int)(r / Cu);
  dw[((size_t)tap * Cin + c_off + c) * N + n] = tmp[(size_t)c * 27 * N + (size_t)tap * N + n];
}
int launch_permute_up_dw(hipStream_t st, const float* tmp, int Cu, int N, int Cin, int c_off, float* dw) {
  const size_t total = (size_t)27 * Cu * N;
  ICS_LAUNCH(permute_up_dw_kernel, dim3((unsigned)((total + 255) / 256)), dim3(256), 0, st, tmp, Cu, N, Cin,
                     c_off, total, dw);
  ICS_HIP(hipGetLastError());
  return 0;
}

__global__ void adam_kernel(float* __restrict__ p, const float* __restrict__ g, float* __restrict__ m,
                            float* __restrict__ v, size_t n, float lr_t, float b1, float b2, float omb1,
                            float omb2, float eps, float gscale) {
  const size_t i = (size_t)blockIdx.x * blockDim.x + threadIdx.x;
  if (i >= n) return;
  const float gi = g[i] * gscale;
  const float mi = b1 * m[i] + omb1 * gi;
  const float vi = b2 * v[i] + omb2 * gi * gi;
  m[i] = mi;
  v[i] = vi;
  p[i] = p[i] - lr_t * mi / (sqrtf(vi) + eps);
}
int launch_adam(hipStream_t st, float* p, const float* g, float* m, float* v, size_t n, float lr_t,
                float gscale) {
  ICS_LAUNCH(adam_kernel, dim3((unsigned)((n + 255) / 256)), dim3(256), 0, st, p, g, m, v, n,
                     lr_t, 0.9f, 0.999f, (float)(1.0 - 0.9), (float)(1.0 - 0.999), 1e-7f, gscale);
  ICS_HIP(hipGetLastError());
  return 0;
}

__global__ void bn_apply_kernel(const float* __restrict__ s, const float* __restrict__ scale,
                                const float* __restrict__ shift, int act, size_t n, int C,
                                float* __restrict__ out) {
  const size_t i = (size_t)blockIdx.x * blockDim.x + threadIdx.x;
  if (i >= n) return;
  const int c = i % C;
  out[i] = act_fwd(scale ? fmaf(s[i], scale[c], shift[c]) : s[i], act);
}
int launch_bn_apply(hipStream_t st, const float* s, const float* scale, const float* shift, int act,
                    size_t n, int C, float* out) {
  ICS_LAUNCH(bn_apply_kernel, dim3((unsigned)((n + 255) / 256)), dim3(256), 0, st, s, scale, shift,
                     act, n, C, out);
  ICS_HIP(hipGetLastError());
  return 0;
}
// ... 286 lines not shown
```

icsg3d_amd/csrc/engine.hip:

```cpp
#include "common.h"
#include "elementwise.h"
#include "segment.h"
#include "scratch.h"
#include "voxelise.h"
#include "latent.h"
#include "tsne.h"
#include "render.h"
#include "monitor.h"
#include "feed.h"
#include "../../include/icsg3d.h"

#include <rccl/rccl.h>
#include <roctracer/roctx.h>

#include <cmath>
#include <cstring>
#include <functional>
#include <map>
#include <memory>
#include <mutex>
#include <vector>

namespace ics {

// ... 94 lines not shown
struct ConvLayer {
  std::string name;
  int Cin = 0, Cout = 0, taps = 27, S = 1;
  int flags = 0;
  bool cond_fold = false;
  float* cond_T = nullptr;
  int bwd_pre_nblk = 0, bwd_pre_ld = 0;
  int CinG = 0;
  float* pad_in = nullptr;
  float* dw_phys = nullptr;
  ConvSrc vsrc[2];
  int nvsrc = 0;
  int pre_act = ACT_NONE, has_bn = 0, post_act = ACT_NONE;
  int Kpad = 0, Npad = 0, Kpad_b = 0, Npad_b = 0;
  int t_w = -1, t_b = -1, t_gamma = -1, t_beta = -1;
  float *mm = nullptr, *mv = nullptr, *mean = nullptr, *rstd = nullptr, *scale = nullptr, *shift = nullptr;
  float *wp = nullptr, *wf = nullptr;
  float *ww = nullptr, *wwb = nullptr;
  int ww_layout = 0, wwb_layout = 0;
  bool wino_w = false;
  int wg_vt_batch = 0;
  float *wg = nullptr, *wgb = nullptr, *wg_v = nullptr, *wg_m = nullptr, *wg_vt = nullptr, *wg_z = nullptr, *wg_du = nullptr;
  bool wg_w = false;
  float* s = nullptr;
  float* dy = nullptr;
  float* dA = nullptr;
  float* c1c2 = nullptr;
  float* db_partial = nullptr;
  int stat_rpb = 0, stat_nblk = 0;
  int db_blocks = 0;
  size_t db_rows = 0;
  float* xs = nullptr;
  float* abc = nullptr;
  bool dy_ready = false;
  unsigned char* tie_mask = nullptr;
  int tie_batch = 0;
  float* tie_ssum = nullptr;
  double* bn_sums = nullptr;
  ConvLayer* skip_prod = nullptr;
  ConvLayer* deferred_skip = nullptr;
  float* pooled = nullptr;
  unsigned char* pool_idx = nullptr;
  ConvSrc src[2];
  int nsrc = 1;
  bool split_up = false;
  bool wf_stale = false;
  int Cs = 0, Cu = 0;
  float *wf_skip = nullptr, *w_up = nullptr;
  float *wp_skip = nullptr, *wp_par = nullptr;
  float* w_up3 = nullptr;
  float* w_up3n = nullptr;
  float *dyS = nullptr;
  int ldS = 0;
  float *dA_skip = nullptr, *dxl = nullptr;
  float *dw_up = nullptr;
};

struct Net {
  int kind = 0;
  int device = 0;
  int flags = 0;
  hipStream_t st = nullptr;
  hipStream_t st2 = nullptr;
  hipEvent_t ev_fork = nullptr, ev_join = nullptr;
  bool side_on = true, side_dirty = false;
  bool pm_side = false;
  int maxB = 0, d = 0, C = 0;
  std::vector<void*> allocs;
  std::vector<Tensor> tensors;
  std::map<std::string, int> tindex;
  size_t nparams = 0;
  float *P = nullptr, *G = nullptr, *Mo = nullptr, *Vo = nullptr;
  int adam_t = 0;
  float lr = 1e-6f;
  bool packed_valid = false;
  void* d_pack_jobs = nullptr;
  int pack_njobs = -1;
  unsigned pack_nblocks = 0;
  int pool_ties_all = 1, bn_unbias = 1;
  int bce_from_logits = 0;
  Profiler prof;
  std::vector<std::unique_ptr<ConvLayer>> layers;
  float* ws_stat = nullptr;  size_t ws_stat_n = 0;
  float* ws_bwd = nullptr;   size_t ws_bwd_n = 0;
  float* ws_bwd2 = nullptr;  size_t ws_bwd2_n = 0;
  float* ws_wgrad = nullptr; size_t ws_wgrad_n = 0;
  float* ws_fwd = nullptr;   size_t ws_fwd_n = 0;
  bool want_tie_stats = false;
  bool want_wgrad_inputs = false;
  bool splitk = false;
  float* fws() const { return splitk ? ws_fwd : nullptr; }
  double* ws_dbl = nullptr;  size_t ws_dbl_n = 0;
  float* d_metrics = nullptr;
  ncclComm_t comm = nullptr;
  ncclComm_t comm_bn = nullptr;
  ncclComm_t small() const { return comm_bn ? comm_bn : comm; }
  int rank = 0, nranks = 1;
  double* d_red = nullptr;
  hipStream_t comm_st = nullptr;
  hipEvent_t ev_grad = nullptr, ev_comm = nullptr;
  size_t bucket_hi = 0, bucket_min = 0;
  int buckets_issued = 0;
  bool overlap = true;
  int sync_bn = 0;
  float* bn_slab = nullptr;
  size_t bn_slab_n = 0, bn_slab_used = 0;
// ... 190 lines not shown
    }
    if (L.has_bn) { ICS_TRY(n.alloc(&L.xs, (size_t)2 * L.Cout)); ICS_TRY(n.alloc(&L.abc, (size_t)3 * L.Cout)); }
  }
  if (L.has_bn) {
    if (!n.bn_slab) {
      size_t tot = 0;
      for (auto& q : n.layers) if (q->has_bn) tot += 2 * (size_t)q->Cout;
      ICS_TRY(n.alloc(&n.bn_slab, tot));
      n.bn_slab_n = tot;
    }
    ICS_CHECK(n.bn_slab_used + 2 * (size_t)L.Cout <= n.bn_slab_n, "BN slab overflow");
    L.mm = n.bn_slab + n.bn_slab_used; L.mv = L.mm + L.Cout;
    n.bn_slab_used += 2 * (size_t)L.Cout;
    n.sync_cmax = std::max(n.sync_cmax, L.Cout);
    ICS_TRY(n.alloc(&L.mean, (size_t)L.Cout)); ICS_TRY(n.alloc(&L.rstd, (size_t)L.Cout));
    ICS_TRY(n.alloc(&L.scale, (size_t)L.Cout)); ICS_TRY(n.alloc(&L.shift, (size_t)L.Cout));
    int ti = n.add_tensor(L.name + "/moving_mean", {L.Cout}, false);
    n.tensors[ti].ptr = L.mm;
    ti = n.add_tensor(L.name + "/moving_var", {L.Cout}, false);
    n.tensors[ti].ptr = L.mv;
  }
  if (L.cond_fold) {
    ICS_TRY(n.alloc(&L.cond_T, (size_t)n.maxB * 27 * L.Cout));
  } else if (L.CinG != L.Cin) {
    ICS_TRY(n.alloc(&L.pad_in, M * L.CinG));
    if (need_bwd) ICS_TRY(n.alloc(&L.dw_phys, (size_t)L.taps * L.CinG * L.Cout));
  }
  if (pooled) {
    ICS_TRY(n.alloc(&L.pooled, M / 8 * L.Cout));
    ICS_TRY(n.alloc(&L.pool_idx, M / 8 * L.Cout));
    if (need_bwd && L.has_bn && L.Cout % 4 == 0) {
      ICS_TRY(n.alloc(&L.tie_mask, M / 8 * L.Cout));
      ICS_TRY(n.alloc(&L.tie_ssum, M / 8 * L.Cout));
      ICS_TRY(n.alloc(&L.bn_sums, (size_t)2 * L.Cout));
    }
  }
  return 0;
}

static ConvSrc src_plain(const float* p, int C) { return ConvSrc{p, nullptr, nullptr, C, 0, ACT_NONE, 0}; }
static ConvSrc src_layer(const ConvLayer& L, int up) {
  if (L.has_bn) return ConvSrc{L.s, L.scale, L.shift, L.Cout, up, L.post_act, 0};
  return ConvSrc{L.s, nullptr, nullptr, L.Cout, up, ACT_NONE, 0};
}

static ConvGeom geom_fwd(const ConvLayer& L, int B) {
  return ConvGeom{B, L.S, ilog2(L.S), L.CinG, L.Cout, L.taps, L.Kpad, L.Npad, L.flags};
}
static ConvGeom geom_bwd(const ConvLayer& L, int B) {
  return ConvGeom{B, L.S, ilog2(L.S), L.Cout, L.CinG, L.taps, L.Kpad_b, L.Npad_b, L.flags};
}

static ConvGeom geom_up_wgrad(const ConvLayer& L, int B) {
  return ConvGeom{B, L.S / 2, ilog2(L.S / 2), L.Cu, 27 * L.Cout, 1, round_up(L.Cu, 32), L.ldS, L.flags};
}
static ConvGeom geom_up_dgrad(const ConvLayer& L, int B) {
  return ConvGeom{B, L.S / 2, ilog2(L.S / 2), L.ldS, L.Cu, 1, L.ldS, round_up(L.Cu, 32), L.flags};
}
static ConvGeom geom_skip_wgrad(const ConvLayer& L, int B) {
  return ConvGeom{B, L.S, ilog2(L.S), L.Cs, L.Cout, L.taps, round_up(L.taps * L.Cs, 32), L.Npad, L.flags};
}
static ConvGeom geom_skip_dgrad(const ConvLayer& L, int B) {
  return ConvGeom{B, L.S, ilog2(L.S), L.Cout, L.Cs, L.taps, L.Kpad_b, round_up(L.Cs, 32), L.flags};
}
static ConvGeom geom_skip_fwd(const ConvLayer& L, int B) {
  return ConvGeom{B, L.S, ilog2(L.S), L.Cs, L.Cout, L.taps, round_up(L.taps * L.Cs, 32), L.Npad, L.flags};
}
static ConvGeom geom_par_fwd(const ConvLayer& L, int B) {
  return ConvGeom{B, L.S / 2, ilog2(L.S / 2), L.Cu, L.Cout, 8, 8 * L.Cu, L.Npad, L.flags};
}
static ConvSrc src_lowres(const ConvLayer& L) { ConvSrc u = L.src[L.nsrc - 1]; u.up = 0; return u; }

static int enable_split_up(Net& n, ConvLayer& L) {
  if (n.flags & CF_NO_UPSPLIT) return 0;
  const ConvSrc& up = L.src[L.nsrc - 1];
  const int Cs = L.nsrc == 2 ? L.src[0].C : 0;
  if (!up.up || (L.nsrc == 2 && L.src[0].up) || L.taps != 27 || L.S < 2 || L.CinG != L.Cin || Cs % 32 || up.C % 32 ||
      up.bcast || L.Cout % 4)
    return 0;
  L.split_up = true;
  L.Cs = Cs; L.Cu = up.C;
  L.ldS = round_up(27 * L.Cout, 32);
  const size_t M = n.rows(L, n.maxB);
  ICS_TRY(n.alloc(&L.w_up, (size_t)L.ldS * round_up(L.Cu, 32)));
  ICS_TRY(n.alloc(&L.dyS, M / 8 * L.ldS));
  ICS_HIP(hipMemsetAsync(L.dyS, 0, M / 8 * L.ldS * sizeof(float), n.st));
  ICS_TRY(n.alloc(&L.dxl, M / 8 * L.Cu));
  ICS_TRY(n.alloc(&L.dw_up, (size_t)L.Cu * 27 * L.Cout));
  if (conv_up3_ok(geom_par_fwd(L, n.maxB), src_lowres(L)))
    ICS_TRY(n.alloc(&L.w_up3, conv_up3_weight_floats(L.Cu, L.Cout)));
  else if (L.Cs == 0 && conv_up3n_ok(geom_par_fwd(L, n.maxB), src_lowres(L)))
    ICS_TRY(n.alloc(&L.w_up3n, conv_up3n_weight_floats(L.Cu, L.Cout)));
  else
    ICS_TRY(n.alloc(&L.wp_par, (size_t)8 * 8 * L.Cu * L.Npad));
  if (L.Cs) {
    ICS_TRY(n.alloc(&L.wf_skip, (size_t)L.Kpad_b * round_up(L.Cs, 32)));
    ICS_TRY(n.alloc(&L.dA_skip, M * L.Cs));
    ICS_TRY(n.alloc(&L.wp_skip, (size_t)round_up(L.taps * L.Cs, 32) * L.Npad));
  }
  return 0;
}

static ConvGeom geom_wino_fwd(const ConvLayer& L, int B) { return L.split_up ? geom_skip_fwd(L, B) : geom_fwd(L, B); }
static ConvGeom geom_wino_bwd(const ConvLayer& L, int B) {
  if (L.split_up) return geom_skip_dgrad(L, B);
  ConvGeom g = geom_bwd(L, B);
  g.Cout = L.Cin;
  return g;
}
static int enable_wino(Net& n, ConvLayer& L, bool need_bwd) {
  if ((n.flags & CF_NO_WINO) || L.taps != 27 || L.pad_in || L.cond_fold || L.CinG != L.Cin) return 0;
  if (L.split_up ? L.Cs == 0 : L.nsrc != 1) return 0;
  const int K = L.split_up ? L.Cs : L.Cin;
  if (conv_wino_ok(geom_wino_fwd(L, n.maxB), L.src, 1)) {
    ICS_TRY(n.alloc(&L.ww, conv_wino_weight_floats(K, L.Cout)));
    L.ww_layout = conv_wino_layout(geom_wino_fwd(L, n.maxB));
  }
  const ConvSrc sdy = src_plain(nullptr, L.Cout);
  if (need_bwd && conv_wino_ok(geom_wino_bwd(L, n.maxB), &sdy, 1)) {
    ICS_TRY(n.alloc(&L.wwb, conv_wino_weight_floats(K, L.Cout)));
    L.wwb_layout = conv_wino_layout(geom_wino_bwd(L, n.maxB));
  }
  L.wino_w = need_bwd && conv_wino_wgrad_ok(L.split_up ? geom_skip_wgrad(L, n.maxB) : geom_fwd(L, n.maxB), L.src, 1);
  return 0;
}

static int enable_winog(Net& n, ConvLayer& L, bool need_bwd) {
  if (L.ww || L.taps != 27 || L.pad_in || L.cond_fold || L.CinG != L.Cin || L.split_up || L.nsrc != 1) return 0;
  const ConvGeom g = geom_fwd(L, n.maxB);
  if (!conv_winog_ok(g, L.src, 1)) return 0;
  size_t v, m, z;
  conv_winog_scratch_floats(g, &v, &m, &z);
  ICS_TRY(n.alloc(&L.wg, conv_winog_weight_floats(L.Cin, L.Cout)));
  ICS_TRY(n.alloc(&L.wg_v, v));
  ICS_TRY(n.alloc(&L.wg_m, m));
  if (need_bwd) {
    ConvGeom gb = geom_bwd(L, n.maxB);
    gb.Cout = L.Cin;
    const ConvSrc sdy = src_plain(nullptr, L.Cout);
    if (conv_winog_ok(gb, &sdy, 1)) ICS_TRY(n.alloc(&L.wgb, conv_winog_weight_floats(L.Cin, L.Cout)));
    L.wg_w = true;
    ICS_TRY(n.alloc(&L.wg_vt, (size_t)64 * n.maxB * 8 * L.Cin));
    ICS_TRY(n.alloc(&L.wg_z, z));
    ICS_TRY(n.alloc(&L.wg_du, (size_t)64 * L.Cin * L.Cout));
  }
  return 0;
}

static int alloc_workspaces(Net& n, bool need_bwd) {
  size_t stat = 0, bwd = 0, wg = 0, fw = 0;
  for (int b = 1; b <= n.maxB; ++b)
  for (auto& Lp : n.layers) {
    ConvLayer& L = *Lp;
    const size_t M = n.rows(L, b);
    const ConvGeom g = geom_fwd(L, b);
    const int rpb = std::min(conv_fwd_rows_per_block(g), 64);
    stat = std::max(stat, (M + rpb - 1) / rpb * 3 * (size_t)L.Npad);
    if (L.split_up) stat = std::max(stat, 8 * ((M / 8 + 63) / 64) * 3 * (size_t)L.Npad);
    fw = std::max(fw, conv_fwd_workspace_floats(g, L.src, L.nsrc));
    if (need_bwd) {
      const ConvSrc sdy = src_plain(L.dy, L.Cout);
      fw = std::max(fw, conv_fwd_workspace_floats(geom_bwd(L, b), &sdy, 1));
      if (L.split_up) {
        const ConvSrc sd = src_plain(L.dyS, L.ldS);
        fw = std::max(fw, conv_fwd_workspace_floats(geom_up_dgrad(L, b), &sd, 1));
        if (L.Cs) fw = std::max(fw, conv_fwd_workspace_floats(geom_skip_dgrad(L, b), &sdy, 1));
      }
      LayerBwd lb{};
      lb.B = b; lb.S = L.S; lb.lgS = ilog2(L.S); lb.C = L.Cout;
      if (&L != n.head) bwd = std::max(bwd, layer_bwd_workspace_floats(lb));
      wg = std::max(wg, conv_wgrad_workspace_floats(g, L.src, L.nsrc));
      if (L.wino_w)
        wg = std::max(wg, conv_wino_wgrad_workspace_floats(L.split_up ? geom_skip_wgrad(L, b) : g));
      if ((L.Cin == 1 || L.cond_fold) && (L.Cout == 16 || L.Cout == 32))
        wg = std::max(wg, conv_thin_c_wgrad_workspace_floats(g));
      if (L.split_up) {
        const ConvSrc lo = src_lowres(L);
        wg = std::max(wg, conv_wgrad_workspace_floats(geom_up_wgrad(L, b), &lo, 1));
        if (L.Cs) wg = std::max(wg, conv_wgrad_workspace_floats(geom_skip_wgrad(L, b), L.src, 1));
      }
    }
  }
  n.ws_stat_n = stat; n.ws_bwd_n = std::max(bwd, (size_t)4096 * 128); n.ws_wgrad_n = wg;
  ICS_TRY(n.alloc(&n.ws_stat, stat + 16));
  n.ws_fwd_n = std::max(fw, (size_t)768 * 64 * 64);
  ICS_TRY(n.alloc(&n.ws_fwd, n.ws_fwd_n + 16));
  if (need_bwd) {
    ICS_TRY(n.alloc(&n.ws_bwd, n.ws_bwd_n + 16));
    ICS_TRY(n.alloc(&n.ws_wgrad, wg + 16));
    size_t b2 = 0;
    for (auto& Lp : n.layers)
      if (Lp->has_bn) b2 = std::max(b2, (size_t)2 * Lp->Npad * ((n.rows(*Lp, n.maxB) + 63) / 64));
    n.ws_bwd2_n = b2;
    ICS_TRY(n.alloc(&n.ws_bwd2, b2 + 16));
    size_t cls = 0; int cmax = 0;
    for (auto& Lp : n.layers)
      if (Lp->taps == 27 && Lp->S >= 3 && Lp->Cout % 4 == 0) {
        for (int b = 1; b <= n.maxB; ++b) cls = std::max(cls, conv_bnfuse_partial_floats(b, Lp->S, Lp->Cout));
        cmax = std::max(cmax, Lp->Cout);
      }
    n.ws_cls_n = cls;
    ICS_TRY(n.alloc(&n.ws_cls, cls + 16));
    ICS_TRY(n.alloc(&n.ws_R, (size_t)48 * cmax + 16));
    size_t pl = 0;
    for (auto& Lp : n.layers)
      if (Lp->tie_mask) pl = std::max(pl, pool_bnfuse_partial_doubles(n.rows(*Lp, n.maxB) / 8, Lp->Cout));
    n.ws_pool_n = pl;
    ICS_TRY(n.alloc(&n.ws_pool, pl + 16));
    if (const char* e = getenv("ICSG3D_DGRAD_BNFUSE_MIN")) n.bnfuse_min_bytes = (size_t)atoll(e);
  }
  n.ws_dbl_n = 1 << 16;
  for (auto& Lp : n.layers)
    if (Lp->cond_fold) n.ws_dbl_n = std::max(n.ws_dbl_n, cond_wgrad_workspace_doubles(n.maxB, Lp->Cout));
  ICS_TRY(n.alloc(&n.ws_dbl, n.ws_dbl_n));
  ICS_TRY(n.alloc(&n.d_metrics, (size_t)16));
  ICS_TRY(n.alloc(&n.d_red, (size_t)16));
  return 0;
// ... 173 lines not shown
static GradSrc gs_pool(const float* p, int ld, const ConvLayer& producer) {
  return GradSrc{p, ld, 0, GS_POOL, producer.pooled, producer.pool_idx};
}

static hipStream_t side_begin(Net& n) {
  if (!n.side_on || (n.prof.on && n.prof.filter.empty())) return n.st;
  (void)hipEventRecord(n.ev_fork, n.st);
  (void)hipStreamWaitEvent(n.st2, n.ev_fork, 0);
  n.side_dirty = true;
  return n.st2;
}
static int side_join(Net& n) {
  if (!n.side_dirty) return 0;
  ICS_HIP(hipEventRecord(n.ev_join, n.st2));
  ICS_HIP(hipStreamWaitEvent(n.st, n.ev_join, 0));
  n.side_dirty = false;
  return 0;
}

static BwdStat bwd_stat_for(Net& n, ConvLayer* next, int B) {
  BwdStat bs;
  if (next == nullptr || !next->has_bn || (n.flags & CF_NO_BWD_FOLD)) return bs;
  if ((size_t)2 * next->Npad * ((n.rows(*next, B) + 63) / 64) > n.ws_bwd2_n) return bs;
  bs.s = next->s; bs.mean = next->mean; bs.rstd = next->rstd; bs.scale = next->scale; bs.shift = next->shift;
  bs.partial = n.ws_bwd2; bs.post_act = next->post_act; bs.ld = next->Cout;
  return bs;
}
static void bwd_stat_done(ConvLayer* next, const BwdStat& bs, int blocks, int npad) {
  if (next == nullptr) return;
  next->bwd_pre_nblk = bs.partial ? blocks : 0;
  next->bwd_pre_ld = npad;
}

static bool skip_bnfuse_ok(const Net& n, const ConvLayer& L, int B) {
  const ConvLayer* P = L.skip_prod;
  if (P == nullptr || !L.split_up || L.Cs == 0 || (n.flags & CF_NO_DGRAD_BNFUSE) || n.sync() != nullptr || n.side_on) return false;
  if (!P->has_bn || P->pre_act != ACT_RELU || P->post_act != ACT_NONE || P->tie_mask == nullptr || P->xs == nullptr ||
      P->db_partial == nullptr || !P->pooled || P->Cout != L.Cs || L.src[0].p != P->s || L.src[0].scale == nullptr ||
      L.src[0].act != ACT_NONE || !n.want_wgrad_inputs || P->tie_batch != B)
    return false;
  if (!L.wino_w || !L.wwb || L.wwb_layout != 1) return false;
  if (n.rows(L, B) * (size_t)P->Cout * sizeof(float) < 2 * n.bnfuse_min_bytes) return false;
  const ConvGeom gw = geom_skip_wgrad(L, B), gd = geom_skip_dgrad(L, B);
  const ConvSrc sdy = src_plain(L.dy, L.Cout);
  return conv_bnfuse_ok(L.S, L.Cs, L.Cout) && conv_wino_wgrad_ok(gw, L.src, 1) && conv_wino_ok(gd, &sdy, 1) &&
         conv_bnfuse_partial_floats(B, L.S, L.Cout) <= n.ws_cls_n && L.Cs % 4 == 0 &&
         pool_bnfuse_partial_doubles(n.rows(L, B) / 8, P->Cout) <= n.ws_pool_n;
}
static int conv_grads_split_up(Net& n, ConvLayer& L, int B, ConvLayer* next) {
  const size_t M = n.rows(L, B);
  const double fl_skip = 2.0 * M * 27 * L.Cs * L.Cout, fl_up = 2.0 * (M / 8) * 27 * L.Cu * L.Cout;
  const bool skipfuse = skip_bnfuse_ok(n, L, B);
  ConvLayer* P = L.skip_prod;
  n.prof.begin(n.st, "pool27:" + L.name, 0, 4.0 * M * L.Cout * (1 + 27.0 / 8));
  ICS_TRY(launch_pool27(n.st, L.dy, B, L.S, L.Cout, L.dyS, L.ldS));
  n.prof.end(n.st);
  hipStream_t ws = side_begin(n);
  if (L.Cs) {
    const ConvGeom g = geom_skip_wgrad(L, B);
    n.prof.begin(ws, "conv_wgrad:" + L.name + ".skip|", fl_skip,
                 4.0 * (M * L.Cs + M * L.Cout + 27.0 * L.Cs * L.Cout));
    const bool wino = L.wino_w && conv_wino_wgrad_ok(g, L.src, 1);
    ConvSrc sx = L.src[0];
    if (skipfuse) { sx.scale = P->xs; sx.shift = P->xs + P->Cout; }
    if (wino)
      ICS_TRY(launch_conv_wgrad_wino(ws, g, sx, L.dy, L.Cout, n.tg(L.t_w), L.Cout, n.ws_wgrad, n.ws_wgrad_n,
                                     L.Cs, L.Cin, 0, 1));
    else
    ICS_TRY(launch_conv_wgrad(ws, g, L.src, 1, L.dy, L.Cout, n.tg(L.t_w), L.Cout, n.ws_wgrad, n.ws_wgrad_n, L.Cs,
                              L.Cin, 0, 1));
    n.prof.end(ws);
    n.prof.begin(ws, "wgrad_reduce_splits", 0, 0);
    if (wino)
      ICS_TRY(launch_conv_wgrad_wino(ws, g, sx, L.dy, L.Cout, n.tg(L.t_w), L.Cout, n.ws_wgrad, n.ws_wgrad_n,
                                     L.Cs, L.Cin, 0, 2));
    else
    ICS_TRY(launch_conv_wgrad(ws, g, L.src, 1, L.dy, L.Cout, n.tg(L.t_w), L.Cout, n.ws_wgrad, n.ws_wgrad_n, L.Cs,
                              L.Cin, 0, 2));
    n.prof.end(ws);
    if (skipfuse) {
      const bool pend = L.db_blocks > 0;
      n.prof.begin(ws, "bnfuse:" + L.name + ".skip", 0, 0);
      ICS_TRY(launch_conv_bnfuse(ws, L.dy, B, L.S, L.Cs, L.Cin, L.Cout, pend ? L.db_partial : n.tg(L.t_b), pend ? L.db_blocks : 1,
                                 n.tp(L.t_w), n.tg(L.t_w), n.tp(P->t_gamma), n.tp(P->t_beta), P->mean, P->rstd, P->scale,
                                 nullptr, nullptr, nullptr, nullptr, n.ws_cls, n.ws_cls_n, n.ws_R, P->bn_sums));
      n.prof.end(ws);
      P->deferred_skip = &L;
    }
  }
  {
    const ConvGeom g = geom_up_wgrad(L, B);
    const ConvSrc lo = src_lowres(L);
    n.prof.begin(ws, "conv_wgrad:" + L.name + ".up|", fl_up,
                 4.0 * (M / 8 * L.Cu + M / 8 * 27.0 * L.Cout + 27.0 * L.Cu * L.Cout));
    ICS_TRY(launch_conv_wgrad(ws, g, &lo, 1, L.dyS, L.ldS, L.dw_up, 27 * L.Cout, n.ws_wgrad, n.ws_wgrad_n, 0, 0, 0, 1));
    n.prof.end(ws);
    n.prof.begin(ws, "wgrad_reduce_splits", 0, 0);
    ICS_TRY(launch_conv_wgrad(ws, g, &lo, 1, L.dyS, L.ldS, L.dw_up, 27 * L.Cout, n.ws_wgrad, n.ws_wgrad_n, 0, 0, 0, 2));
    ICS_TRY(launch_permute_up_dw(ws, L.dw_up, L.Cu, L.Cout, L.Cin, L.Cs, n.tg(L.t_w)));
    n.prof.end(ws);
  }
  if (L.Cs && !skipfuse) {
    const ConvGeom g = geom_skip_dgrad(L, B);
    ConvSrc sdy = src_plain(L.dy, L.Cout);
    n.prof.begin(n.st, "conv_dgrad:" + L.name + ".skip|", fl_skip,
                 4.0 * (M * L.Cs + M * L.Cout + 27.0 * L.Cs * L.Cout));
    if (L.wwb && conv_wino_ok(g, &sdy, 1))
      ICS_TRY(launch_conv_fwd_wino(n.st, g, sdy, L.wwb, nullptr, L.dA_skip, L.Cs, ACT_NONE, nullptr, nullptr, 0,
                                   L.wwb_layout));
    else
    ICS_TRY(launch_conv_fwd(n.st, g, &sdy, 1, L.wf_skip, nullptr, L.dA_skip, L.Cs, ACT_NONE, nullptr, nullptr, 0,
                            n.fws(), n.ws_fwd_n));
    n.prof.end(n.st);
  }
  {
    const ConvGeom g = geom_up_dgrad(L, B);
    ConvSrc sd = src_plain(L.dyS, L.ldS);
    n.prof.begin(n.st, "conv_dgrad:" + L.name + ".up|", fl_up,
                 4.0 * (M / 8 * L.Cu + M / 8 * 27.0 * L.Cout + 27.0 * L.Cu * L.Cout));
    const BwdStat bs = bwd_stat_for(n, next, B);
    int blocks = 0;
    ICS_TRY(launch_conv_fwd(n.st, g, &sd, 1, L.w_up, nullptr, L.dxl, L.Cu, ACT_NONE, nullptr, nullptr, 0, n.fws(),
                            n.ws_fwd_n, &bs, &blocks));
    bwd_stat_done(next, bs, blocks, g.Npad);
    n.prof.end(n.st);
  }
  return 0;
}

static int colsum_push(Net& n, const float* partial, int nblk, int C, float* out);
static bool dgrad_bnfuse_ok(const Net& n, const ConvLayer& L, const ConvLayer* next, int B, bool need_dA, bool param_grads) {
  if (next == nullptr || !need_dA || !param_grads || (n.flags & CF_NO_DGRAD_BNFUSE) || n.sync() != nullptr || n.side_on)
    return false;
  if (!next->has_bn || next->pre_act != ACT_RELU || next->post_act != ACT_NONE || next->xs == nullptr ||
      next->db_partial == nullptr || next->dy == nullptr)
    return false;
  if (L.split_up || L.nsrc != 1 || L.taps != 27 || !L.wino_w || !L.wwb || L.CinG != L.Cin ||
      L.Cin != next->Cout || L.src[0].p != next->s || L.src[0].scale == nullptr || L.src[0].act != ACT_NONE || L.dw_phys)
    return false;
  if (n.rows(L, B) * (size_t)next->Cout * sizeof(float) < n.bnfuse_min_bytes) return false;
  const ConvGeom g = geom_fwd(L, B);
  ConvGeom gb = geom_bwd(L, B);
  gb.Cout = L.Cin;
  const ConvSrc sdy = src_plain(L.dy, L.Cout);
  return conv_bnfuse_ok(L.S, L.Cin, L.Cout) && conv_wino_wgrad_ok(g, L.src, 1) && conv_wino_ok(gb, &sdy, 1) &&
         conv_bnfuse_partial_floats(B, L.S, L.Cout) <= n.ws_cls_n && L.Cin % 4 == 0;
}
static int conv_grads_from_dy(Net& n, ConvLayer& L, int B, bool need_dA, bool param_grads, ConvLayer* next) {
  if (L.split_up && need_dA && param_grads) return conv_grads_split_up(n, L, B, next);
  if (L.split_up) next = nullptr;
  const ConvGeom g = geom_fwd(L, B);
  const size_t M = n.rows(L, B);
  const bool bnfuse = dgrad_bnfuse_ok(n, L, next, B, need_dA, param_grads);
  if (param_grads) {
    hipStream_t ws = side_begin(n);
    n.prof.begin(ws, "conv_wgrad:" + L.name + "|", 2.0 * M * L.taps * L.Cin * L.Cout,
                 4.0 * (M * L.Cin + M * L.Cout + (double)L.taps * L.Cin * L.Cout));
    float* dw = L.dw_phys ? L.dw_phys : n.tg(L.t_w);
    const bool thin1 = L.pad_in && L.nvsrc == 1 && L.Cin == 1 && conv_thin_c_ok(g, L.vsrc[0], 1, 1) && L.Cout % 4 == 0;
    if (L.cond_fold) {
      const ConvSrc& cs = L.vsrc[1];
      const int C0 = L.vsrc[0].C;
      ICS_TRY(launch_conv_wgrad_thin_c(ws, g, L.vsrc[0], L.dy, L.Cout, n.tg(L.t_w), L.Cout, L.Cin, n.ws_wgrad,
                                       n.ws_wgrad_n, 0));
      ICS_TRY(launch_cond_wgrad(ws, L.dy, B, L.S, L.Cout, cs.p, C0, cs.C, cs.bcast, L.Cin, n.tg(L.t_w), n.ws_dbl,
                                n.ws_dbl_n));
      conv_set_last_kernel_id(L.Cout == 32 ? "conv_thin_c_wgrad_kernel<32> + cond_wgrad_kernel"
                                           : "conv_thin_c_wgrad_kernel<16> + cond_wgrad_kernel");
      n.prof.end(ws);
    } else if (thin1) {
// ... 2238 lines not shown
  auto down = [&](float* host, const float* dev, size_t cnt) -> int {
    if (host) ICS_HIP(hipMemcpyAsync(host, dev, cnt * sizeof(float), hipMemcpyDeviceToHost, n.st));
    return 0;
  };
  ICS_TRY(down(a->y, L.s, M * Cout));
  a->rows_per_block = 0; a->blocks = 0;
  if (a->has_bn) {
    ICS_TRY(down(a->mean, L.mean, Cout)); ICS_TRY(down(a->rstd, L.rstd, Cout));
    ICS_TRY(down(a->scale, L.scale, Cout)); ICS_TRY(down(a->shift, L.shift, Cout));
    ICS_TRY(down(a->moving_mean, L.mm, Cout)); ICS_TRY(down(a->moving_var, L.mv, Cout));
    a->rows_per_block = L.stat_rpb; a->blocks = L.stat_nblk;
  }
  std::vector<float> hA;
  if (bwd) {
    ICS_TRY(down(a->dw, n.tg(L.t_w), wn)); ICS_TRY(down(a->dbias, n.tg(L.t_b), Cout));
    if (a->has_bn) { ICS_TRY(down(a->dgamma, n.tg(L.t_gamma), Cout)); ICS_TRY(down(a->dbeta, n.tg(L.t_beta), Cout)); }
    if (want_dx && L.split_up) {
      if (L.Cs) ICS_TRY(down(a->src[0].dx, L.dA_skip, M * L.Cs));
      ICS_TRY(down(a->src[a->nsrc - 1].dx, L.dxl, M / 8 * L.Cu));
    } else if (want_dx) {
      hA.resize(M * L.CinG);
      ICS_TRY(down(hA.data(), L.dA, hA.size()));
    }
  }
  ICS_HIP(hipStreamSynchronize(n.st));
  n.prof.resolve();
  if (!hA.empty()) {
    int c0 = 0;
    const int ld = L.CinG, h = S / 2;
    for (int i = 0; i < a->nsrc; c0 += a->src[i].C, ++i) {
      const ics_conv_layer_src& s = a->src[i];
      if (!s.dx) continue;
      if (!s.up) {
        for (size_t m = 0; m < M; ++m)
          for (int c = 0; c < s.C; ++c) s.dx[m * s.C + c] = hA[m * ld + c0 + c];
        continue;
      }
      for (int b = 0; b < B; ++b)
        for (int z = 0; z < h; ++z)
          for (int y = 0; y < h; ++y)
            for (int x = 0; x < h; ++x) {
              float* o = s.dx + ((((size_t)b * h + z) * h + y) * h + x) * s.C;
              for (int c = 0; c < s.C; ++c) o[c] = 0.f;
              for (int k = 0; k < 8; ++k) {
                const size_t m = (((size_t)b * S + 2 * z + (k >> 2)) * S + 2 * y + ((k >> 1) & 1)) * S + 2 * x + (k & 1);
                for (int c = 0; c < s.C; ++c) o[c] += hA[m * ld + c0 + c];
              }
            }
    }
  }
  if (a->kernels && a->kernels_cap > 0) {
    std::string txt;
    for (const auto& r : n.prof.rows)
      if (r.label.find('|') != std::string::npos) txt += r.label + "\n";
    std::strncpy(a->kernels, txt.c_str(), (size_t)a->kernels_cap - 1);
    a->kernels[a->kernels_cap - 1] = 0;
  }
  if (n.canary_on) {
    std::string msg;
    const int bad = n.canaries_dirty(&msg);
    ICS_CHECK(bad == 0, op + "guard bytes written behind " + std::to_string(bad) + " buffer(s): " + msg);
  }
  return 0;
}
int ics_op_conv_layer(ics_conv_layer* a) {
  const std::string op = "ics_op_conv_layer: ";
  ICS_CHECK(a != nullptr, op + "null argument");
  ICS_CHECK(a->ranks >= 0 && a->ranks <= 4, op + "ranks must be in [0, 4]");
  ICS_TRY(conv_layer_check(a, op));
  if (a->ranks == 0) return conv_layer_body(a, nullptr);
  int Cin = 0;
  for (int i = 0; i < a->nsrc; ++i) Cin += a->src[i].C;
  const size_t M = (size_t)a->B * a->S * a->S * a->S, C = (size_t)a->Cout, wn = (size_t)a->taps * Cin * C;
  auto body = [&](int r, BnSyncEmu* emu) -> int {
    ics_conv_layer v = *a;
    auto off = [r](float*& p, size_t cnt) { if (p) p += (size_t)r * cnt; };
    for (int i = 0; i < v.nsrc; ++i) {
      const size_t cnt = v.src[i].bcast > 0 ? (size_t)a->B * v.src[i].bcast : (v.src[i].up ? M / 8 : M) * v.src[i].C;
      v.src[i].x += (size_t)r * cnt;
      off(v.src[i].dx, cnt);
    }
    if (v.dout) v.dout += (size_t)r * M * C;
    off(v.y, M * C);
    off(v.mean, C); off(v.rstd, C); off(v.scale, C); off(v.shift, C); off(v.moving_mean, C); off(v.moving_var, C);
    off(v.dw, wn); off(v.dbias, C); off(v.dgamma, C); off(v.dbeta, C);
    if (v.kernels) v.kernels += (size_t)r * (v.kernels_cap > 0 ? v.kernels_cap : 0);
    ICS_TRY(conv_layer_body(&v, emu));
    a->rows_per_block = v.rows_per_block; a->blocks = v.blocks;
    return 0;
  };
  return run_emulated_ranks(op, a->ranks, a->Cout, 2, body);
}

static int conv_link_check(const ics_conv_link* a, const std::string& op) {
  ICS_CHECK(a->link >= ICS_LINK_SAME && a->link <= ICS_LINK_POOL_SKIP, op + "unknown link");
  ICS_CHECK(a->form == 0 || a->form == 1, op + "form must be 0 (U-Net) or 1 (VAE)");
  ICS_CHECK(a->B >= 1 && a->max_batch >= a->B, op + "need 1 <= B <= max_batch");
  const bool has_k = a->link == ICS_LINK_POOL || a->link == ICS_LINK_POOL_SKIP, has_l = a->link != ICS_LINK_POOL;
  const bool skip = a->link == ICS_LINK_POOL_SKIP;
  ICS_CHECK(a->S >= (has_k ? 2 : 1) && (a->S & (a->S - 1)) == 0, op + "S must be a power of two (>= 2 in front of a pool)");
  ICS_CHECK(a->C0 >= 1 && a->x0 != nullptr, op + "x0 and C0 are required");
  ICS_CHECK(a->dout != nullptr, op + "dout is required");
  ICS_CHECK(!skip || (a->q != nullptr && a->Cq >= 1 && a->dout_l != nullptr), op + "POOL_SKIP needs q, Cq and dout_l");
  ICS_CHECK(a->pool_ties_all == 0 || a->pool_ties_all == 1, op + "pool_ties_all must be 0 or 1");
  ICS_CHECK(has_k || a->pooled == nullptr, op + "pooled needs a pool link");
  auto layer_ok = [](const ics_conv_link_layer& l) { return l.Cout >= 1 && l.w && l.gamma && l.beta; };
  ICS_CHECK(layer_ok(a->P), op + "P needs Cout, w, gamma and beta");
// ... 508 lines not shown
```

icsg3d_amd/engine.py:

```python
from __future__ import annotations

import ctypes as C

import numpy as np

from . import _lib as L


def _f32(a):
    return np.ascontiguousarray(a, dtype=np.float32)


def _jobs4(jobs):
    jobs = np.ascontiguousarray(jobs, np.int32)
    if jobs.ndim != 2 or jobs.shape[1] != 4:
        raise ValueError("jobs must be (B, 4) int32 {structure, r0, r1, r2}, got %s" % (jobs.shape,))
    return jobs


class _Net:

    def __init__(self):
        self._h = L._H(None)
        self._lib = L.load()
# ... 666 lines not shown
    taps, Cout = w.shape[0] ** 3, w.shape[4]
    srcs = [dict(s) for s in sources]
    x0 = _f32(srcs[0]["x"])
    NB = x0.shape[0]
    if NB % max(R, 1):
        raise ValueError("the batch does not divide into %d equal shards" % R)
    B = NB // max(R, 1)
    S = x0.shape[1] * (2 if srcs[0].get("up") else 1)
    if sum(int(s["C"]) if s.get("bcast") else _f32(s["x"]).shape[4] for s in srcs) != w.shape[3]:
        raise ValueError("the sources' channels do not add up to the kernel's Cin")
    a.B, a.max_batch, a.S, a.taps, a.Cout = B, int(max_batch or B), S, taps, Cout
    a.pre_act, a.has_bn, a.post_act, a.pad_input, a.nsrc = int(pre_act), int(bool(has_bn)), int(post_act), int(bool(pad_input)), len(srcs)
    dxs = []
    for i, s in enumerate(srcs):
        x = _f32(s["x"])
        up = 1 if s.get("up") else 0
        bcast = int(s.get("bcast", 0))
        if bcast:
            if x.shape != (NB, bcast):
                raise ValueError("source %d has shape %s, a bcast source is (B, bcast)" % (i, x.shape))
        elif x.shape[:4] != (NB,) + (S // 2 if up else S,) * 3:
            raise ValueError("source %d has shape %s" % (i, x.shape))
        a.src[i].x, a.src[i].scale, a.src[i].shift = f(x), f(s.get("scale")), f(s.get("shift"))
        a.src[i].C, a.src[i].up, a.src[i].act = int(s["C"]) if bcast else x.shape[4], up, int(s.get("act", 0))
        a.src[i].bcast = bcast
        if bcast:
            dxs.append(None)
        elif dout is not None and want_dx:
            dxs.append(out(x.shape))
            a.src[i].dx = L.fptr(dxs[-1])
    a.w, a.bias, a.gamma, a.beta, a.dout = f(w), f(bias), f(gamma), f(beta), f(dout)
    r = {"y": out((NB, S, S, S, Cout))}
    a.y = L.fptr(r["y"])
    if has_bn:
        for k in ("mean", "rstd", "scale", "shift", "moving_mean", "moving_var"):
            r[k] = out(lead + (Cout,))
            setattr(a, k, L.fptr(r[k]))
    if dout is not None:
        r["dw"], r["dbias"] = out(lead + w.shape), out(lead + (Cout,))
        a.dw, a.dbias = L.fptr(r["dw"]), L.fptr(r["dbias"])
        if has_bn:
            r["dgamma"], r["dbeta"] = out(lead + (Cout,)), out(lead + (Cout,))
            a.dgamma, a.dbeta = L.fptr(r["dgamma"]), L.fptr(r["dbeta"])
        r["dx"] = dxs
    cap = 16384
    text = C.create_string_buffer(cap * max(R, 1))
    a.kernels, a.kernels_cap = C.cast(text, C.c_void_p), cap
    L.check(lib.ics_op_conv_layer(C.byref(a)))
    if has_bn:
        r["rows_per_block"], r["blocks"] = a.rows_per_block, a.blocks

    def kernels(i):
        lines = text.raw[i * cap:(i + 1) * cap].split(b"\0", 1)[0].decode().splitlines()
        return {k: [ln for ln in lines if ln.startswith("conv_%s:" % k)] for k in ("fwd", "dgrad", "wgrad")}

    r["kernels"] = [kernels(i) for i in range(R)] if R else kernels(0)
    return r


LINKS = ("same", "up", "pool", "pool_skip")
METRIC_SUM_KEYS = ("sum_lsoft", "sum_lsig", "tp", "predicted", "wr_tp", "wr_possible", "voxels")


def conv_link(link, x0, layers, dout, form="unet", q=None, dout_l=None, pool_ties_all=True, max_batch=None, ranks=0):
    lib = L.load()
    R = int(ranks)
    if not 0 <= R <= 4:
        raise ValueError("ranks must be in 0..4")
    lead = (R,) if R else ()
    a = L.ConvLinkArgs()
    a.ranks = R
    keep = []

    def f(v):
        if v is None:
            return None
        v = _f32(v)
        keep.append(v)
        return L.fptr(v)

    def out(shape):
        v = np.empty(shape, np.float32)
        keep.append(v)
        return v

    x0 = _f32(x0)
    NB, S, C0 = x0.shape[0], x0.shape[1], x0.shape[4]
    if NB % max(R, 1):
        raise ValueError("the batch does not divide into %d equal shards" % R)
    B = NB // max(R, 1)
    a.link, a.form = LINKS.index(link), {"unet": 0, "vae": 1}[form]
    a.B, a.max_batch, a.S, a.C0 = B, int(max_batch or B), S, C0
    a.pool_ties_all = int(bool(pool_ties_all))
    a.x0, a.q, a.dout, a.dout_l = f(x0), f(q), f(dout), f(dout_l)
    a.Cq = 0 if q is None else _f32(q).shape[4]
    side = {"P": S, "K": S // 2, "L": 2 * S if link == "up" else S}
    r = {}
    for name, p in layers.items():
        h = getattr(a, name)
        w = _f32(p["w"])
        Cout = w.shape[4]
        h.Cout, h.w, h.bias, h.gamma, h.beta = Cout, f(w), f(p.get("bias")), f(p["gamma"]), f(p["beta"])
        o = r[name] = {"y": out((NB,) + (side[name],) * 3 + (Cout,)), "dw": out(lead + w.shape)}
        for k in ("mean", "rstd", "scale", "shift", "dbias", "dgamma", "dbeta"):
            o[k] = out(lead + (Cout,))
        for k, v in o.items():
            setattr(h, k, L.fptr(v))
# ... 121 lines not shown
```

Before: 1148.

## Store upsample backward pool sums as eight shifted volumes instead of 27 taps

Adds an UP8 layout in which the pooled upsample gradient is kept as 8 half-resolution volumes, each padded by one voxel. The 27 tap views become address offsets into these volumes, replacing the 27x-expanded pool27 buffer. The forward (dgrad) and wgrad GEMM kernels get an UP8 template path that computes row and chunk addresses from the new geometry, and a pool8 kernel fills the volumes. This is meant to cut the memory traffic and footprint of the 27-tap materialisation, at the cost of more complex address arithmetic and restrictions on shape and tile.

```diff
diff --git a/icsg3d_amd/csrc/common.h b/icsg3d_amd/csrc/common.h
--- a/icsg3d_amd/csrc/common.h
+++ b/icsg3d_amd/csrc/common.h
@@ -6,6 +6,8 @@
 #include <cstdio>
 #include <string>
 #include <vector>
+
+#include "up8.h"
 
 namespace ics {
 
@@ -106,6 +108,8 @@
   CF_NO_DGRAD_BNFUSE = 1 << 22,
   CF_NO_POOL_PRESUM = 1 << 23,
   CF_NO_HEAD_LABELS = 1 << 24,
+  CF_NO_UP8 = 1 << 25,
+  CF_UP8 = 1 << 26,
   CF_ZBATCH = 1 << 20,
 };
 int conv_flags_from_env();
@@ -140,6 +144,7 @@
                     float* splitk_ws = nullptr, size_t splitk_ws_floats = 0, const BwdStat* bwd = nullptr,
                     int* bwd_blocks = nullptr);
 size_t conv_fwd_workspace_floats(const ConvGeom& g, const ConvSrc* src, int nsrc);
+bool conv_fwd_up8_tile_ok(const ConvGeom& g);
 bool conv_thin_c_ok(const ConvGeom& g, const ConvSrc& s0, int nsrc, int cin_log);
 size_t conv_thin_c_wgrad_workspace_floats(const ConvGeom& g);
 int launch_conv_wgrad_thin_c(hipStream_t st, const ConvGeom& g, const ConvSrc& s0, const float* dy, int ldy, float* dw,
diff --git a/icsg3d_amd/csrc/conv_igemm.hip b/icsg3d_amd/csrc/conv_igemm.hip
--- a/icsg3d_amd/csrc/conv_igemm.hip
+++ b/icsg3d_amd/csrc/conv_igemm.hip
@@ -60,6 +60,7 @@
   if (getenv("ICSG3D_NO_DGRAD_BNFUSE")) f |= CF_NO_DGRAD_BNFUSE;
   if (getenv("ICSG3D_NO_POOL_PRESUM")) f |= CF_NO_POOL_PRESUM;
   if (getenv("ICSG3D_NO_HEAD_LABELS")) f |= CF_NO_HEAD_LABELS;
+  if (getenv("ICSG3D_NO_UP8")) f |= CF_NO_UP8;
   { const char* e = getenv("ICSG3D_UP3_BIG_MIN_WG"); if (e && *e && strtoul(e, nullptr, 10) <= 1) f |= CF_UP3_BIG_ALWAYS; }
   return f;
 }
@@ -176,13 +177,13 @@
 }
 
 template <int WM, int WN, int TM, int TN, bool VEC, int ABL = 0, bool AFF = true, bool UP = true, bool THIN = false,
-          bool REUSE = false, bool PAR = false, bool NOACT = false, bool FOLD = false>
+          bool REUSE = false, bool PAR = false, bool NOACT = false, bool FOLD = false, bool UP8 = false>
 __global__ __launch_bounds__(256, FOLD ? 2 : ((REUSE && PAR) ? 3 : 1)) void conv_fwd_kernel(ConvGeom g, ConvSrc s0, ConvSrc s1,
                                                         const float* __restrict__ wp,
                                                         const float* __restrict__ bias,
                                                         float* __restrict__ out, int ldo, int pre_act,
                                                         float* __restrict__ stat_partial, int gridM,
-                                                        int gridN, int accumulate, BwdStat bs) {
+                                                        int gridN, int accumulate, BwdStat bs, Up8Geom u8) {
   constexpr int BM = WM * TM * 32, BN = WN * TN * 32;
   constexpr int B_FLOATS = 32 * BN;
   constexpr int RA = BM / 32;
@@ -407,16 +408,18 @@
 #pragma unroll
     for (int r = 0; r < RA; ++r) {
       const unsigned mc = (unsigned)min(mrow_base + 32 * r, M - 1);
-      rowG0[r] = (mc * (unsigned)s0.C + (unsigned)(t & 7) * 4u) * 4u;
+      rowG0[r] = UP8 ? (up8_row_floats(mc, u8) + (unsigned)(t & 7) * 4u) * 4u
+                     : (mc * (unsigned)s0.C + (unsigned)(t & 7) * 4u) * 4u;
       rowG1[r] = (mc * (unsigned)s1.C + (unsigned)(t & 7) * 4u) * 4u;
     }
   }
   auto load_chunk_gemm = [&](int c) {
     load_b(c * 8);
     const int ci0 = c << 5;
-    const bool first = ci0 < s0.C;
+    const bool first = UP8 || ci0 < s0.C;
     const int cbase = first ? ci0 : ci0 - s0.C;
-    const char* sp = reinterpret_cast<const char*>(first ? s0.p : s1.p) + (size_t)cbase * 4;
+    const char* sp = UP8 ? reinterpret_cast<const char*>(s0.p) + up8_chunk_floats(c, u8) * 4
+                         : reinterpret_cast<const char*>(first ? s0.p : s1.p) + (size_t)cbase * 4;
     const float slope = first ? slope0 : slope1;
     v4f sc = v4f{1.f, 1.f, 1.f, 1.f}, sh = v4f{0.f, 0.f, 0.f, 0.f};
     if (AFF) {
@@ -596,8 +599,9 @@
 #pragma unroll
         for (int r = 0; r < NB; ++r) xb[r] = *reinterpret_cast<const v4f*>(wrow + bofs[r]);
         const int ci0 = c << 5;
-        const bool first = ci0 < s0.C;
-        const char* sp = reinterpret_cast<const char*>(first ? s0.p : s1.p) + (size_t)(first ? ci0 : ci0 - s0.C) * 4;
+        const bool first = UP8 || ci0 < s0.C;
+        const char* sp = UP8 ? reinterpret_cast<const char*>(s0.p) + up8_chunk_floats(c, u8) * 4
+                             : reinterpret_cast<const char*>(first ? s0.p : s1.p) + (size_t)(first ? ci0 : ci0 - s0.C) * 4;
 #pragma unroll
         for (int r = 0; r < RA; ++r) xa[r] = *reinterpret_cast<const v4f*>(sp + (first ? rowG0[r] : rowG1[r]));
       };
@@ -815,7 +819,7 @@
 }
 
 template <int WM, int WN, int TM, int TN, bool VEC, int ABL = 0, bool AFF = true, bool UP = true, bool THIN = false,
-          bool REUSE = false, bool PAR = false, bool NOACT = false, bool FOLD = false>
+          bool REUSE = false, bool PAR = false, bool NOACT = false, bool FOLD = false, bool UP8 = false>
 static int launch_fwd_cfg(hipStream_t st, const ConvGeom& g, const ConvSrc& s0, const ConvSrc& s1,
                           const float* wp, const float* bias, float* out, int ldo, int pre_act,
                           float* stat_partial, int* rows_per_block, int accumulate = 0, int ksplit = 1,
@@ -825,7 +829,7 @@
   const int gridM = (M + BM - 1) / BM, gridN = g.Npad / BN;
   const int arows = REUSE ? BM + (BM >> g.lgS) + 1 : BM;
   const size_t lds = (size_t)(arows * kLDA + 2 * 32 * BN) * sizeof(float);
-  auto kern = conv_fwd_kernel<WM, WN, TM, TN, VEC, ABL, AFF, UP, THIN, REUSE, PAR, NOACT, FOLD>;
+  auto kern = conv_fwd_kernel<WM, WN, TM, TN, VEC, ABL, AFF, UP, THIN, REUSE, PAR, NOACT, FOLD, UP8>;
   static DevOnce attr;
   int dev;
   if (attr.need(&dev)) {
@@ -838,12 +842,14 @@
   static const std::string id = std::string("conv_fwd_kernel<") + std::to_string(WM) + ", " + std::to_string(WN) + ", " +
                                 std::to_string(TM) + ", " + std::to_string(TN) + ", " + tf(VEC) + ", " +
                                 std::to_string(ABL) + ", " + tf(AFF) + ", " + tf(UP) + ", " + tf(THIN) + ", " +
-                                tf(REUSE) + ", " + tf(PAR) + ", " + tf(NOACT) + ", " + tf(FOLD) + ">";
+                                tf(REUSE) + ", " + tf(PAR) + ", " + tf(NOACT) + ", " + tf(FOLD) + (UP8 ? ", UP8>" : ">");
   g_last_kernel_id = id.c_str();
   BwdStat bs_arg;
   if (FOLD) bs_arg = *bwd;
+  Up8Geom u8;
+  if (UP8) u8 = up8_geom(g.B, g.S, g.lgS, g.Cin / 27);
   ICS_LAUNCH(kern, dim3(gridM * gridN, PAR ? 8 : 1, ksplit), dim3(256), lds, st, g, s0, s1, wp, bias, out, ldo,
-                     pre_act, stat_partial, gridM, gridN, accumulate, bs_arg);
+                     pre_act, stat_partial, gridM, gridN, accumulate, bs_arg, u8);
   ICS_HIP(hipGetLastError());
   return 0;
 }
@@ -858,6 +864,13 @@
   }
   *bm = BM;
   *bn = BN;
+}
+
+static bool up8_tile(int bm, int bn) { return bm == 64 || bn == 128 || bn == 64; }
+bool conv_fwd_up8_tile_ok(const ConvGeom& g) {
+  int bm, bn;
+  pick_fwd_tile(g, &bm, &bn);
+  return up8_tile(bm, bn);
 }
 
 static bool fwd_is_vec(const ConvGeom& g, const ConvSrc& s0, const ConvSrc& s1) {
@@ -1698,6 +1711,22 @@
   int bm, bn;
   pick_fwd_tile(g, &bm, &bn);
 #define ICS_FWD_ARGS st, g, s0, s1, wp, bias, out, ldo, pre_act, stat_partial, rows_per_block, accumulate, ksplit, bwd
+  if (g.flags & CF_UP8) {
+    ICS_CHECK(vec && !thin && variant == 0 && nsrc == 1 && g.taps == 1 && g.Cin % 27 == 0 && g.Kpad == g.Cin &&
+                  up8_shape_ok(2 * g.S, g.Cin / 27, (size_t)g.B << (3 * g.lgS), g.B),
+              "up8 backward-data: shape outside the 8-volume layout");
+#define ICS_FWD8(WM, WN, TM, TN)                                                                                     \
+  do {                                                                                                               \
+    if (fold)                                                                                                        \
+      return launch_fwd_cfg<WM, WN, TM, TN, true, 0, false, false, false, false, false, false, true, true>(ICS_FWD_ARGS); \
+    return launch_fwd_cfg<WM, WN, TM, TN, true, 0, false, false, false, false, false, false, false, true>(ICS_FWD_ARGS); \
+  } while (0)
+    ICS_CHECK(up8_tile(bm, bn), "up8 backward-data: no UP8 instantiation of this tile");
+    if (bm == 64) { ICS_FWD8(2, 2, 1, 1); }
+    if (bn == 128) { ICS_FWD8(2, 2, 2, 2); }
+    ICS_FWD8(2, 2, 2, 1);
+#undef ICS_FWD8
+  }
 #define ICS_FWD(WM, WN, TM, TN)                                                                 \
   do {                                                                                          \
     if (thin) return launch_fwd_cfg<WM, WN, TM, TN, true, 0, true, true, true>(ICS_FWD_ARGS);   \
@@ -1862,12 +1891,12 @@
 
 
 template <int WM, int WN, int TM, int TN, bool VEC, bool DYVEC, bool AFF = true, bool UP = true, bool THIN = false,
-          int ABL = 0>
+          int ABL = 0, bool UP8 = false>
 __global__ __launch_bounds__(256) void conv_wgrad_kernel(ConvGeom g, ConvSrc s0, ConvSrc s1,
                                                           const float* __restrict__ dy, int ldy,
                                                           int n_load,
                                                           float* __restrict__ ws, int ktiles,
-                                                          int ntiles, int rows_per_split) {
+                                                          int ntiles, int rows_per_split, Up8Geom u8) {
   constexpr int KT = WM * TM * 32, NT = WN * TN * 32;
   constexpr int A_FLOATS = 32 * KT, D_FLOATS = 32 * NT;
   constexpr int AF4 = KT / 4, ATOT = 32 * AF4, APASS = ATOT / 256;
@@ -1985,7 +2014,7 @@
     }
   };
   const bool gemm = VEC && DYVEC && !UP && !THIN && ABL == 0 && g.taps == 1 && (M & 31) == 0 &&
-                    (rows_per_split & 31) == 0 && n0 + NT <= n_load;
+                    (rows_per_split & 31) == 0 && (UP8 || n0 + NT <= n_load);
   const bool noact_g = slope == 1.f;
   unsigned aoffg[VEC ? APASS : 1], doffg[DPASS];
   if (VEC) {
@@ -1995,13 +2024,16 @@
 #pragma unroll
   for (int p = 0; p < DPASS; ++p) {
     const int idx = t + 256 * p;
-    doffg[p] = (unsigned)((idx / DF4) * ldy + n0 + (idx % DF4) * 4) * 4u;
+    doffg[p] = UP8 ? (up8_prow((unsigned)(idx / DF4), u8.lgSh, u8.P) * (unsigned)u8.N +
+                      up8_col_floats(min(n0 + (idx % DF4) * 4, n_load - 4), u8)) * 4u
+                   : (unsigned)((idx / DF4) * ldy + n0 + (idx % DF4) * 4) * 4u;
   }
   auto load_chunk_gemm = [&](int c, auto noact_tag) {
     constexpr bool NA = decltype(noact_tag)::value;
     const int mbase = m_begin + (c << 5);
     const char* abase = reinterpret_cast<const char*>(sp) + (size_t)mbase * (size_t)sC * 4;
-    const char* dbase = reinterpret_cast<const char*>(dy) + (size_t)mbase * (size_t)ldy * 4;
+    const char* dbase = reinterpret_cast<const char*>(dy) +
+                        (UP8 ? up8_chunk_base_floats((unsigned)mbase, u8) : (size_t)mbase * (size_t)ldy) * 4;
     if (VEC) {
 #pragma unroll
       for (int p = 0; p < APASS; ++p) {
@@ -2088,7 +2120,8 @@
     auto loadS = [&](int c, v4f (&xa)[APASS], v4f (&xd)[DPASS]) {
       const int mbase = m_begin + (c << 5);
       const char* abase = reinterpret_cast<const char*>(sp) + (size_t)mbase * (size_t)sC * 4;
-      const char* dbase = reinterpret_cast<const char*>(dy) + (size_t)mbase * (size_t)ldy * 4;
+      const char* dbase = reinterpret_cast<const char*>(dy) +
+                        (UP8 ? up8_chunk_base_floats((unsigned)mbase, u8) : (size_t)mbase * (size_t)ldy) * 4;
 #pragma unroll
       for (int p = 0; p < APASS; ++p) xa[p] = *reinterpret_cast<const v4f*>(abase + aoffg[p]);
 #pragma unroll
@@ -2648,12 +2681,12 @@
 }
 
 template <int WM, int WN, int TM, int TN, bool VEC, bool DYVEC, bool AFF = true, bool UP = true, bool THIN = false,
-          int ABL = 0>
+          int ABL = 0, bool UP8 = false>
 static int launch_wgrad_cfg(hipStream_t st, const ConvGeom& g, const ConvSrc& s0, const ConvSrc& s1,
                             const float* dy, int ldy, int n_load, float* ws, const WgradPlan& p) {
   constexpr int KT = WM * TM * 32, NT = WN * TN * 32;
   const size_t lds = (size_t)2 * 32 * (KT + NT) * sizeof(float);
-  auto kern = conv_wgrad_kernel<WM, WN, TM, TN, VEC, DYVEC, AFF, UP, THIN, ABL>;
+  auto kern = conv_wgrad_kernel<WM, WN, TM, TN, VEC, DYVEC, AFF, UP, THIN, ABL, UP8>;
   static DevOnce attr;
   int dev;
   if (attr.need(&dev)) {
@@ -2664,10 +2697,12 @@
   static const std::string id = std::string("conv_wgrad_kernel<") + std::to_string(WM) + ", " + std::to_string(WN) +
                                 ", " + std::to_string(TM) + ", " + std::to_string(TN) + ", " + tf(VEC) + ", " +
                                 tf(DYVEC) + ", " + tf(AFF) + ", " + tf(UP) + ", " + tf(THIN) + ", " +
-                                std::to_string(ABL) + ">";
+                                std::to_string(ABL) + (UP8 ? ", UP8>" : ">");
   g_last_kernel_id = id.c_str();
+  Up8Geom u8;
+  if (UP8) u8 = up8_geom(g.B, g.S, g.lgS, g.Cout / 27);
   ICS_LAUNCH(kern, dim3(p.ktiles * p.ntiles * p.ksplit), dim3(256), lds, st, g, s0, s1, dy,
-                     ldy, n_load, ws, p.ktiles, p.ntiles, p.rows_per_split);
+                     ldy, n_load, ws, p.ktiles, p.ntiles, p.rows_per_split, u8);
   ICS_HIP(hipGetLastError());
   return 0;
 }
@@ -2813,7 +2848,21 @@
     else if (aff) ICS_TRY((launch_wgrad_cfg<WM, WN, TM, TN, true, DV, true, false>(ICS_WG_ARGS))); \
     else ICS_TRY((launch_wgrad_cfg<WM, WN, TM, TN, true, DV, false, false>(ICS_WG_ARGS)));         \
   } while (0)
-  if (!dy_vec) {
+  if (g.flags & CF_UP8) {
+    const int M8 = g.B << (3 * g.lgS);
+    ICS_CHECK(dy_vec && p.vec && !p.thin && !up && g.taps == 1 && g.Cout % 27 == 0 && n_load == g.Cout && M8 % 32 == 0 &&
+                  p.rows_per_split % 32 == 0 && up8_shape_ok(2 * g.S, g.Cout / 27, (size_t)M8, g.B),
+              "up8 backward-weight: shape outside the 8-volume layout");
+#define ICS_WG8(WM, WN, TM, TN)                                                                                  \
+  do {                                                                                                           \
+    if (aff) ICS_TRY((launch_wgrad_cfg<WM, WN, TM, TN, true, true, true, false, false, 0, true>(ICS_WG_ARGS)));  \
+    else ICS_TRY((launch_wgrad_cfg<WM, WN, TM, TN, true, true, false, false, false, 0, true>(ICS_WG_ARGS)));     \
+  } while (0)
+    ICS_CHECK(p.nt == 128 && p.kt >= 64, "up8 backward-weight: no UP8 instantiation of this tile");
+    if (p.kt == 128) ICS_WG8(2, 2, 2, 2);
+    else ICS_WG8(2, 2, 1, 2);
+#undef ICS_WG8
+  } else if (!dy_vec) {
     if (p.kt == 128) ICS_WG(4, 1, 1, 1, false);
     else if (p.kt == 64) ICS_WG(2, 2, 1, 1, false);
     else ICS_WG(1, 4, 1, 1, false);
diff --git a/icsg3d_amd/csrc/elementwise.h b/icsg3d_amd/csrc/elementwise.h
--- a/icsg3d_amd/csrc/elementwise.h
+++ b/icsg3d_amd/csrc/elementwise.h
@@ -141,6 +141,7 @@
 int launch_colsum_small(hipStream_t st, const float* a, int rows, int cols, int ld, float* out);
 int launch_axpy(hipStream_t st, float* y, const float* x, size_t n, float a);
 int launch_pool27(hipStream_t st, const float* dy, int B, int S, int N, float* out, int ldo);
+int launch_pool8(hipStream_t st, const float* dy, int B, int S, int N, float* out, const Up8Geom& u);
 int launch_permute_up_dw(hipStream_t st, const float* tmp, int Cu, int N, int Cin, int c_off, float* dw);
 
 }
diff --git a/icsg3d_amd/csrc/elementwise.hip b/icsg3d_amd/csrc/elementwise.hip
--- a/icsg3d_amd/csrc/elementwise.hip
+++ b/icsg3d_amd/csrc/elementwise.hip
@@ -1839,6 +1839,63 @@
   ICS_HIP(hipGetLastError());
   return 0;
 }
+__global__ __launch_bounds__(256) void pool8_kernel(const float* __restrict__ dy, int B, int S, int N, size_t total,
+                                                    float* __restrict__ out, Up8Geom u) {
+  const size_t i = (size_t)blockIdx.x * blockDim.x + threadIdx.x;
+  if (i >= total) return;
+  const int Sh = S >> 1, N4 = N >> 2, P = u.P;
+  const int n = (int)(i % N4) * 4;
+  size_t r = i / N4;
+  const int jx = r % P; r /= P;
+  const int jy = r % P; r /= P;
+  const int jz = r % P;
+  const int b = (int)(r / P);
+  pf4 o[2][2][2];
+#pragma unroll
+  for (int k = 0; k < 8; ++k) o[k >> 2][(k >> 1) & 1][k & 1] = pf4{0.f, 0.f, 0.f, 0.f};
+#pragma unroll
+  for (int sz = 0; sz < 3; ++sz) {
+    const int z = 2 * jz - 1 + sz;
+    if ((unsigned)z >= (unsigned)S) continue;
+    pf4 lx[3][2];
+#pragma unroll
+    for (int sy = 0; sy < 3; ++sy) {
+      const int y = 2 * jy - 1 + sy;
+      pf4 v[3];
+#pragma unroll
+      for (int sx = 0; sx < 3; ++sx) {
+        const int x = 2 * jx - 1 + sx;
+        const bool ok = (unsigned)y < (unsigned)S && (unsigned)x < (unsigned)S;
+        v[sx] = ok ? *reinterpret_cast<const pf4*>(dy + ((((size_t)b * S + z) * S + y) * S + x) * N + n) : pf4{0.f, 0.f, 0.f, 0.f};
+      }
+      lx[sy][1] = v[0] + v[1];
+      lx[sy][0] = v[1] + v[2];
+    }
+#pragma unroll
+    for (int kx = 0; kx < 2; ++kx) {
+      const pf4 q = lx[0][kx] + lx[1][kx], rr = lx[1][kx] + lx[2][kx];
+      if (sz <= 1) o[1][1][kx] += q;
+      if (sz <= 1) o[1][0][kx] += rr;
+      if (sz >= 1) o[0][1][kx] += q;
+      if (sz >= 1) o[0][0][kx] += rr;
+    }
+  }
+  const size_t row = (((size_t)b * P + jz) * P + jy) * P + jx;
+#pragma unroll
+  for (int k = 0; k < 8; ++k) {
+    const int kz = k >> 2, ky = (k >> 1) & 1, kx = k & 1;
+    if ((kz == 0 && jz == Sh) || (ky == 0 && jy == Sh) || (kx == 0 && jx == Sh)) continue;
+    *reinterpret_cast<pf4*>(out + (size_t)k * u.vstride + row * N + n) = o[kz][ky][kx];
+  }
+}
+int launch_pool8(hipStream_t st, const float* dy, int B, int S, int N, float* out, const Up8Geom& u) {
+  ICS_CHECK(N % 4 == 0 && u.P == S / 2 + 1 && u.N == N && (size_t)u.vstride == up8_volume_floats(B, S / 2, N),
+            "pool8: layout does not match the shape");
+  const size_t total = (size_t)B * u.P * u.P * u.P * (N / 4);
+  ICS_LAUNCH(pool8_kernel, dim3((unsigned)((total + 255) / 256)), dim3(256), 0, st, dy, B, S, N, total, out, u);
+  ICS_HIP(hipGetLastError());
+  return 0;
+}
 __global__ void permute_up_dw_kernel(const float* __restrict__ tmp, int Cu, int N, int Cin, int c_off,
                                      size_t total, float* __restrict__ dw) {
   const size_t i = (size_t)blockIdx.x * blockDim.x + threadIdx.x;
diff --git a/icsg3d_amd/csrc/engine.hip b/icsg3d_amd/csrc/engine.hip
--- a/icsg3d_amd/csrc/engine.hip
+++ b/icsg3d_amd/csrc/engine.hip
@@ -170,6 +170,8 @@
   float* w_up3n = nullptr;
   float *dyS = nullptr;
   int ldS = 0;
+  bool up8 = false;
+  float *dy8 = nullptr;
   float *dA_skip = nullptr, *dxl = nullptr;
   float *dw_up = nullptr;
 };
@@ -466,10 +468,10 @@
 }
 
 static ConvGeom geom_up_wgrad(const ConvLayer& L, int B) {
-  return ConvGeom{B, L.S / 2, ilog2(L.S / 2), L.Cu, 27 * L.Cout, 1, round_up(L.Cu, 32), L.ldS, L.flags};
+  return ConvGeom{B, L.S / 2, ilog2(L.S / 2), L.Cu, 27 * L.Cout, 1, round_up(L.Cu, 32), L.ldS, L.flags | (L.up8 ? CF_UP8 : 0)};
 }
 static ConvGeom geom_up_dgrad(const ConvLayer& L, int B) {
-  return ConvGeom{B, L.S / 2, ilog2(L.S / 2), L.ldS, L.Cu, 1, L.ldS, round_up(L.Cu, 32), L.flags};
+  return ConvGeom{B, L.S / 2, ilog2(L.S / 2), L.ldS, L.Cu, 1, L.ldS, round_up(L.Cu, 32), L.flags | (L.up8 ? CF_UP8 : 0)};
 }
 static ConvGeom geom_skip_wgrad(const ConvLayer& L, int B) {
   return ConvGeom{B, L.S, ilog2(L.S), L.Cs, L.Cout, L.taps, round_up(L.taps * L.Cs, 32), L.Npad, L.flags};
@@ -484,6 +486,15 @@
   return ConvGeom{B, L.S / 2, ilog2(L.S / 2), L.Cu, L.Cout, 8, 8 * L.Cu, L.Npad, L.flags};
 }
 static ConvSrc src_lowres(const ConvLayer& L) { ConvSrc u = L.src[L.nsrc - 1]; u.up = 0; return u; }
+
+static bool up8_ok(const Net& n, const ConvLayer& L) {
+  if (n.flags & CF_NO_UP8) return false;
+  const size_t S3 = (size_t)(L.S / 2) * (L.S / 2) * (L.S / 2);
+  if (L.Cout % 32 || L.Cu % 64 || !up8_shape_ok(L.S, L.Cout, (size_t)n.maxB * S3, n.maxB)) return false;
+  for (int b = 1; b <= n.maxB; ++b)
+    if (!conv_fwd_up8_tile_ok(geom_up_dgrad(L, b))) return false;
+  return true;
+}
 
 static int enable_split_up(Net& n, ConvLayer& L) {
   if (n.flags & CF_NO_UPSPLIT) return 0;
@@ -497,8 +508,15 @@
   L.ldS = round_up(27 * L.Cout, 32);
   const size_t M = n.rows(L, n.maxB);
   ICS_TRY(n.alloc(&L.w_up, (size_t)L.ldS * round_up(L.Cu, 32)));
-  ICS_TRY(n.alloc(&L.dyS, M / 8 * L.ldS));
-  ICS_HIP(hipMemsetAsync(L.dyS, 0, M / 8 * L.ldS * sizeof(float), n.st));
+  L.up8 = up8_ok(n, L);
+  if (L.up8) {
+    const size_t n8 = 8 * up8_volume_floats(n.maxB, L.S / 2, L.Cout);
+    ICS_TRY(n.alloc(&L.dy8, n8));
+    ICS_HIP(hipMemsetAsync(L.dy8, 0, n8 * sizeof(float), n.st));
+  } else {
+    ICS_TRY(n.alloc(&L.dyS, M / 8 * L.ldS));
+    ICS_HIP(hipMemsetAsync(L.dyS, 0, M / 8 * L.ldS * sizeof(float), n.st));
+  }
   ICS_TRY(n.alloc(&L.dxl, M / 8 * L.Cu));
   ICS_TRY(n.alloc(&L.dw_up, (size_t)L.Cu * 27 * L.Cout));
   if (conv_up3_ok(geom_par_fwd(L, n.maxB), src_lowres(L)))
@@ -576,7 +594,7 @@
       const ConvSrc sdy = src_plain(L.dy, L.Cout);
       fw = std::max(fw, conv_fwd_workspace_floats(geom_bwd(L, b), &sdy, 1));
       if (L.split_up) {
-        const ConvSrc sd = src_plain(L.dyS, L.ldS);
+        const ConvSrc sd = src_plain(L.up8 ? L.dy8 : L.dyS, L.ldS);
         fw = std::max(fw, conv_fwd_workspace_floats(geom_up_dgrad(L, b), &sd, 1));
         if (L.Cs) fw = std::max(fw, conv_fwd_workspace_floats(geom_skip_dgrad(L, b), &sdy, 1));
       }
@@ -856,8 +874,15 @@
   const double fl_skip = 2.0 * M * 27 * L.Cs * L.Cout, fl_up = 2.0 * (M / 8) * 27 * L.Cu * L.Cout;
   const bool skipfuse = skip_bnfuse_ok(n, L, B);
   ConvLayer* P = L.skip_prod;
-  n.prof.begin(n.st, "pool27:" + L.name, 0, 4.0 * M * L.Cout * (1 + 27.0 / 8));
-  ICS_TRY(launch_pool27(n.st, L.dy, B, L.S, L.Cout, L.dyS, L.ldS));
+  const float* dyp = L.up8 ? L.dy8 : L.dyS;
+  if (L.up8) {
+    const double pr = (double)(L.S / 2 + 1) / (L.S / 2);
+    n.prof.begin(n.st, "pool8:" + L.name, 0, 4.0 * M * L.Cout * (1 + pr * pr * pr));
+    ICS_TRY(launch_pool8(n.st, L.dy, B, L.S, L.Cout, L.dy8, up8_geom(B, L.S / 2, ilog2(L.S / 2), L.Cout)));
+  } else {
+    n.prof.begin(n.st, "pool27:" + L.name, 0, 4.0 * M * L.Cout * (1 + 27.0 / 8));
+    ICS_TRY(launch_pool27(n.st, L.dy, B, L.S, L.Cout, L.dyS, L.ldS));
+  }
   n.prof.end(n.st);
   hipStream_t ws = side_begin(n);
   if (L.Cs) {
@@ -897,10 +922,10 @@
     const ConvSrc lo = src_lowres(L);
     n.prof.begin(ws, "conv_wgrad:" + L.name + ".up|", fl_up,
                  4.0 * (M / 8 * L.Cu + M / 8 * 27.0 * L.Cout + 27.0 * L.Cu * L.Cout));
-    ICS_TRY(launch_conv_wgrad(ws, g, &lo, 1, L.dyS, L.ldS, L.dw_up, 27 * L.Cout, n.ws_wgrad, n.ws_wgrad_n, 0, 0, 0, 1));
+    ICS_TRY(launch_conv_wgrad(ws, g, &lo, 1, dyp, L.ldS, L.dw_up, 27 * L.Cout, n.ws_wgrad, n.ws_wgrad_n, 0, 0, 0, 1));
     n.prof.end(ws);
     n.prof.begin(ws, "wgrad_reduce_splits", 0, 0);
-    ICS_TRY(launch_conv_wgrad(ws, g, &lo, 1, L.dyS, L.ldS, L.dw_up, 27 * L.Cout, n.ws_wgrad, n.ws_wgrad_n, 0, 0, 0, 2));
+    ICS_TRY(launch_conv_wgrad(ws, g, &lo, 1, dyp, L.ldS, L.dw_up, 27 * L.Cout, n.ws_wgrad, n.ws_wgrad_n, 0, 0, 0, 2));
     ICS_TRY(launch_permute_up_dw(ws, L.dw_up, L.Cu, L.Cout, L.Cin, L.Cs, n.tg(L.t_w)));
     n.prof.end(ws);
   }
@@ -919,7 +944,7 @@
   }
   {
     const ConvGeom g = geom_up_dgrad(L, B);
-    ConvSrc sd = src_plain(L.dyS, L.ldS);
+    ConvSrc sd = src_plain(dyp, L.ldS);
     n.prof.begin(n.st, "conv_dgrad:" + L.name + ".up|", fl_up,
                  4.0 * (M / 8 * L.Cu + M / 8 * 27.0 * L.Cout + 27.0 * L.Cu * L.Cout));
     const BwdStat bs = bwd_stat_for(n, next, B);
@@ -3264,7 +3289,8 @@
   if (a->kernels && a->kernels_cap > 0) {
     std::string txt;
     for (const auto& r : n.prof.rows)
-      if (r.label.find('|') != std::string::npos) txt += r.label + "\n";
+      if (r.label.find('|') != std::string::npos || r.label.rfind("pool8:", 0) == 0 || r.label.rfind("pool27:", 0) == 0)
+        txt += r.label + "\n";
     std::strncpy(a->kernels, txt.c_str(), (size_t)a->kernels_cap - 1);
     a->kernels[a->kernels_cap - 1] = 0;
   }
diff --git a/icsg3d_amd/csrc/hoststub/up8_check.cpp b/icsg3d_amd/csrc/hoststub/up8_check.cpp
--- /dev/null
+++ b/icsg3d_amd/csrc/hoststub/up8_check.cpp
@@ -0,0 +1,209 @@
+#include "../up8.h"
+
+#include <cstdint>
+#include <cstdio>
+#include <cstdlib>
+#include <cstring>
+#include <vector>
+
+static int g_fail = 0;
+#define CHECK(cond, ...)                         \
+  do {                                           \
+    if (!(cond)) {                               \
+      if (g_fail < 20) {                         \
+        fprintf(stderr, "up8_check FAILED: ");   \
+        fprintf(stderr, __VA_ARGS__);            \
+        fprintf(stderr, "\n");                   \
+      }                                          \
+      ++g_fail;                                  \
+    }                                            \
+  } while (0)
+
+static int ilog2i(int v) { int l = 0; while ((1 << l) < v) ++l; return l; }
+
+struct Pos { int vol; size_t row; };
+static Pos expected_pos(int m, int tap, int Sh, int P) {
+  const int x = m % Sh, y = (m / Sh) % Sh, z = (m / (Sh * Sh)) % Sh, b = m / (Sh * Sh * Sh);
+  const int d[3] = {tap / 9 - 1, (tap / 3) % 3 - 1, tap % 3 - 1};
+  const int a[3] = {z, y, x};
+  int slot[3], typ[3];
+  for (int i = 0; i < 3; ++i) {
+    typ[i] = d[i] == 0 ? 0 : 1;
+    slot[i] = d[i] < 0 ? a[i] + 1 : a[i];
+  }
+  return Pos{typ[0] * 4 + typ[1] * 2 + typ[2], (((size_t)b * P + slot[0]) * P + slot[1]) * P + slot[2]};
+}
+
+static void check_addresses(int maxB, int B, int S, int N) {
+  const int Sh = S / 2, lg = ilog2i(Sh), P = Sh + 1;
+  const int M8 = B * Sh * Sh * Sh;
+  CHECK(up8_shape_ok(S, N, (size_t)M8, B), "shape (B %d, S %d, N %d) refused", B, S, N);
+  const Up8Geom u = up8_geom(B, Sh, lg, N);
+  const size_t alloc = 8 * up8_volume_floats(maxB, Sh, N);
+  const size_t vs = u.vstride;
+  CHECK(vs == up8_volume_floats(B, Sh, N) && 8 * vs <= alloc, "volume stride");
+  CHECK(8 * vs * 4 <= 0xffffffffull, "byte offsets exceed 32 bits");
+  const int cpt = N / 32;
+  for (int m = 0; m < M8; ++m) {
+    const uint64_t rowb = ((uint64_t)up8_row_floats((unsigned)m, u) + 28) * 4;
+    CHECK(rowb <= 0xffffffffull, "row byte offset exceeds 32 bits");
+    for (int tap = 0; tap < 27; ++tap) {
+      const Pos e = expected_pos(m, tap, Sh, P);
+      for (int cc = 0; cc < cpt; ++cc) {
+        const size_t off = up8_chunk_floats(tap * cpt + cc, u) + up8_row_floats((unsigned)m, u);
+        const size_t want = (size_t)e.vol * vs + e.row * N + (size_t)cc * 32;
+        CHECK(off == want, "dgrad B %d S %d N %d m %d tap %d cc %d: %zu != %zu", B, S, N, m, tap, cc, off, want);
+        CHECK(off >= (size_t)e.vol * vs && off + 32 <= (size_t)(e.vol + 1) * vs && off + 32 <= alloc,
+              "dgrad B %d S %d N %d m %d tap %d: outside its volume", B, S, N, m, tap);
+      }
+    }
+  }
+  CHECK(M8 % 32 == 0, "whole chunks");
+  for (int mbase = 0; mbase < M8; mbase += 32) {
+    const size_t cb = up8_chunk_base_floats((unsigned)mbase, u);
+    for (int r = 0; r < 32; ++r) {
+      const unsigned pr = up8_prow((unsigned)r, lg, P) * (unsigned)N;
+      for (int n = 0; n < 27 * N; n += 4) {
+        const uint64_t tb = ((uint64_t)pr + up8_col_floats(n, u)) * 4;
+        CHECK(tb <= 0xffffffffull, "per-thread byte offset exceeds 32 bits");
+        const size_t off = cb + pr + up8_col_floats(n, u);
+        const int tap = n / N;
+        const Pos e = expected_pos(mbase + r, tap, Sh, P);
+        const size_t want = (size_t)e.vol * vs + e.row * N + (size_t)(n % N);
+        CHECK(off == want, "wgrad B %d S %d N %d m %d n %d: %zu != %zu", B, S, N, mbase + r, n, off, want);
+        CHECK(off >= (size_t)e.vol * vs && off + 4 <= (size_t)(e.vol + 1) * vs && off + 4 <= alloc,
+              "wgrad B %d S %d N %d m %d n %d: outside its volume", B, S, N, mbase + r, n);
+      }
+    }
+  }
+}
+
+static void pool27_host(const std::vector<float>& dy, int B, int S, int N, std::vector<float>& out) {
+  const int Sh = S / 2;
+  out.assign((size_t)B * Sh * Sh * Sh * 27 * N, 0.f);
+  for (int b = 0; b < B; ++b) for (int a = 0; a < Sh; ++a) for (int bq = 0; bq < Sh; ++bq) for (int c = 0; c < Sh; ++c)
+  for (int n = 0; n < N; ++n) {
+    float o[27];
+    for (int k = 0; k < 27; ++k) o[k] = 0.f;
+    for (int sz = 0; sz < 4; ++sz) {
+      const int z = 2 * a - 1 + sz;
+      if (z < 0 || z >= S) continue;
+      float lx[4][3];
+      for (int sy = 0; sy < 4; ++sy) {
+        const int y = 2 * bq - 1 + sy;
+        float v[4];
+        for (int sx = 0; sx < 4; ++sx) {
+          const int x = 2 * c - 1 + sx;
+          const bool ok = y >= 0 && y < S && x >= 0 && x < S;
+          v[sx] = ok ? dy[((((size_t)b * S + z) * S + y) * S + x) * N + n] : 0.f;
+        }
+        lx[sy][2] = v[0] + v[1]; lx[sy][1] = v[1] + v[2]; lx[sy][0] = v[2] + v[3];
+      }
+      float Pq[3][3];
+      for (int dx = 0; dx < 3; ++dx) {
+        Pq[2][dx] = lx[0][dx] + lx[1][dx]; Pq[1][dx] = lx[1][dx] + lx[2][dx]; Pq[0][dx] = lx[2][dx] + lx[3][dx];
+      }
+      for (int dyi = 0; dyi < 3; ++dyi) for (int dx = 0; dx < 3; ++dx) {
+        if (sz <= 1) o[2 * 9 + dyi * 3 + dx] += Pq[dyi][dx];
+        if (sz >= 1 && sz <= 2) o[1 * 9 + dyi * 3 + dx] += Pq[dyi][dx];
+        if (sz >= 2) o[0 * 9 + dyi * 3 + dx] += Pq[dyi][dx];
+      }
+    }
+    const size_t vl = (((size_t)b * Sh + a) * Sh + bq) * Sh + c;
+    for (int k = 0; k < 27; ++k) out[(vl * 27 + k) * N + n] = o[k];
+  }
+}
+static void pool8_host(const std::vector<float>& dy, int B, int S, int N, const Up8Geom& u, float* out) {
+  const int Sh = S / 2, P = u.P;
+  for (int b = 0; b < B; ++b) for (int jz = 0; jz < P; ++jz) for (int jy = 0; jy < P; ++jy) for (int jx = 0; jx < P; ++jx)
+  for (int n = 0; n < N; ++n) {
+    float o[2][2][2] = {};
+    for (int sz = 0; sz < 3; ++sz) {
+      const int z = 2 * jz - 1 + sz;
+      if (z < 0 || z >= S) continue;
+      float lx[3][2];
+      for (int sy = 0; sy < 3; ++sy) {
+        const int y = 2 * jy - 1 + sy;
+        float v[3];
+        for (int sx = 0; sx < 3; ++sx) {
+          const int x = 2 * jx - 1 + sx;
+          const bool ok = y >= 0 && y < S && x >= 0 && x < S;
+          v[sx] = ok ? dy[((((size_t)b * S + z) * S + y) * S + x) * N + n] : 0.f;
+        }
+        lx[sy][1] = v[0] + v[1]; lx[sy][0] = v[1] + v[2];
+      }
+      for (int kx = 0; kx < 2; ++kx) {
+        const float q = lx[0][kx] + lx[1][kx], rr = lx[1][kx] + lx[2][kx];
+        if (sz <= 1) { o[1][1][kx] += q; o[1][0][kx] += rr; }
+        if (sz >= 1) { o[0][1][kx] += q; o[0][0][kx] += rr; }
+      }
+    }
+    const size_t row = (((size_t)b * P + jz) * P + jy) * P + jx;
+    for (int k = 0; k < 8; ++k) {
+      const int kz = k >> 2, ky = (k >> 1) & 1, kx = k & 1;
+      if ((kz == 0 && jz == Sh) || (ky == 0 && jy == Sh) || (kx == 0 && jx == Sh)) continue;
+      out[(size_t)k * u.vstride + row * N + n] = o[kz][ky][kx];
+    }
+  }
+}
+
+static void check_values(int maxB, int B, int S, int N) {
+  const int Sh = S / 2, lg = ilog2i(Sh), P = Sh + 1, M8 = B * Sh * Sh * Sh;
+  const Up8Geom u = up8_geom(B, Sh, lg, N);
+  std::vector<float> dy((size_t)B * S * S * S * N);
+  uint32_t st = 12345u + (uint32_t)(B * 131 + S * 7 + N);
+  for (auto& v : dy) {
+    st = st * 1664525u + 1013904223u;
+    v = ((int)(st >> 8) % 20001 - 10000) * 1.37e-4f;
+    if ((st >> 28) == 0) v = -0.f;
+  }
+  std::vector<float> ref;
+  pool27_host(dy, B, S, N, ref);
+  const size_t alloc = 8 * up8_volume_floats(maxB, Sh, N);
+  float* vol = (float*)malloc(alloc * sizeof(float));
+  const uint32_t fill = 0x7fc0dead;
+  for (size_t i = 0; i < alloc; ++i) memcpy(vol + i, &fill, 4);
+  pool8_host(dy, B, S, N, u, vol);
+  const int cpt = N / 32;
+  for (int m = 0; m < M8; ++m)
+    for (int tap = 0; tap < 27; ++tap)
+      for (int ch = 0; ch < N; ++ch) {
+        const size_t off = up8_chunk_floats(tap * cpt + ch / 32, u) + up8_row_floats((unsigned)m, u) + ch % 32;
+        const size_t offw = up8_chunk_base_floats((unsigned)(m & ~31), u) + up8_prow((unsigned)(m & 31), lg, P) * (size_t)N +
+                            up8_col_floats(tap * N + ch, u);
+        CHECK(off == offw, "value check: the two loaders disagree at m %d tap %d ch %d", m, tap, ch);
+        const float a = vol[off], b = ref[((size_t)m * 27 + tap) * N + ch];
+        CHECK(memcmp(&a, &b, 4) == 0, "value B %d S %d m %d tap %d ch %d: %.9g != %.9g", B, S, m, tap, ch, a, b);
+      }
+  size_t untouched = 0, expect_untouched = alloc - 8 * (size_t)u.vstride;
+  for (int k = 0; k < 8; ++k) {
+    const int q = (k >> 2) + ((k >> 1) & 1) + (k & 1);
+    size_t used = (size_t)B * N;
+    for (int i = 0; i < 3; ++i) used *= (size_t)(i < q ? P : Sh);
+    expect_untouched += (size_t)u.vstride - used;
+  }
+  for (size_t i = 0; i < alloc; ++i) untouched += memcmp(vol + i, &fill, 4) == 0;
+  CHECK(untouched == expect_untouched, "B %d S %d: %zu untouched floats, expected %zu", B, S, untouched, expect_untouched);
+  free(vol);
+}
+
+int main() {
+  const int Bs[4] = {1, 2, 3, 5}, Ss[4] = {8, 16, 32, 64};
+  long cases = 0;
+  for (int bi = 0; bi < 4; ++bi)
+    for (int si = 0; si < 4; ++si)
+      for (int B = 1; B <= Bs[bi]; ++B) {
+        if (B != Bs[bi] && B != Bs[bi] - 1 && B != 1) continue;
+        check_addresses(Bs[bi], B, Ss[si], Ss[si] >= 32 ? 32 : 64);
+        if (Ss[si] <= 16) { check_addresses(Bs[bi], B, Ss[si], 32); check_values(Bs[bi], B, Ss[si], 32); }
+        if (Ss[si] == 8) check_values(Bs[bi], B, Ss[si], 64);
+        ++cases;
+      }
+  CHECK(!up8_shape_ok(4, 64, 3 * 8, 3), "S = 4 accepted");
+  CHECK(!up8_shape_ok(8, 16, 2 * 64, 2), "N = 16 accepted");
+  CHECK(!up8_shape_ok(16, 96, 512, 1), "N = 96 accepted");
+  CHECK(!up8_shape_ok(64, 512, (size_t)64 * 32768, 64), "a buffer past 4 GiB accepted");
+  if (g_fail) { fprintf(stderr, "up8_check: %d checks FAILED\n", g_fail); return 1; }
+  printf("up8_check: %ld (max_batch, batch, S) cases OK\n", cases);
+  return 0;
+}
diff --git a/icsg3d_amd/csrc/up8.h b/icsg3d_amd/csrc/up8.h
--- /dev/null
+++ b/icsg3d_amd/csrc/up8.h
@@ -0,0 +1,75 @@
+#pragma once
+#include <stddef.h>
+
+#if defined(__HIPCC__) || defined(__CUDACC__)
+#define ICS_UP8_HD __host__ __device__ inline
+#else
+#define ICS_UP8_HD inline
+#endif
+
+struct Up8Geom {
+  int P = 0;
+  int lgSh = 0;
+  int N = 0;
+  int lgcpt = 0;
+  unsigned vstride = 0;
+  unsigned tapoff[27] = {};
+};
+
+struct Up8Tap {
+  int vol;
+  int shift;
+};
+
+ICS_UP8_HD Up8Tap up8_tap(int tap, int P) {
+  const int dz = tap / 9 - 1, dy = (tap / 3) % 3 - 1, dx = tap % 3 - 1;
+  const int vol = (dz != 0 ? 4 : 0) + (dy != 0 ? 2 : 0) + (dx != 0 ? 1 : 0);
+  const int shift = ((dz < 0 ? 1 : 0) * P + (dy < 0 ? 1 : 0)) * P + (dx < 0 ? 1 : 0);
+  return Up8Tap{vol, shift};
+}
+
+ICS_UP8_HD unsigned up8_prow(unsigned m, int lgSh, int P) {
+  const unsigned mask = (1u << lgSh) - 1u;
+  const unsigned x = m & mask, y = (m >> lgSh) & mask, z = (m >> (2 * lgSh)) & mask, b = m >> (3 * lgSh);
+  return ((b * (unsigned)P + z) * (unsigned)P + y) * (unsigned)P + x;
+}
+
+ICS_UP8_HD size_t up8_volume_floats(int B, int Sh, int N) {
+  const size_t P = (size_t)Sh + 1;
+  return (size_t)B * P * P * P * (size_t)N;
+}
+
+ICS_UP8_HD Up8Geom up8_geom(int B, int Sh, int lgSh, int N) {
+  Up8Geom u;
+  u.P = Sh + 1;
+  u.lgSh = lgSh;
+  u.N = N;
+  int l = 0;
+  while ((32 << l) < N) ++l;
+  u.lgcpt = l;
+  u.vstride = (unsigned)up8_volume_floats(B, Sh, N);
+  for (int t = 0; t < 27; ++t) {
+    const Up8Tap tp = up8_tap(t, u.P);
+    u.tapoff[t] = (unsigned)tp.vol * u.vstride + (unsigned)tp.shift * (unsigned)N;
+  }
+  return u;
+}
+
+ICS_UP8_HD bool up8_shape_ok(int S, int N, size_t M8, int B) {
+  if (S < 8 || (S & (S - 1)) != 0 || N < 32 || (N & (N - 1)) != 0 || M8 % 32 != 0) return false;
+  return 8 * up8_volume_floats(B, S / 2, N) * sizeof(float) <= 0xffffffffull;
+}
+
+ICS_UP8_HD size_t up8_chunk_floats(int c, const Up8Geom& u) {
+  const int tap = c >> u.lgcpt, cc = c & ((1 << u.lgcpt) - 1);
+  return (size_t)(u.tapoff[tap] + (unsigned)cc * 32u);
+}
+ICS_UP8_HD unsigned up8_row_floats(unsigned m, const Up8Geom& u) { return up8_prow(m, u.lgSh, u.P) * (unsigned)u.N; }
+
+ICS_UP8_HD unsigned up8_col_floats(int n, const Up8Geom& u) {
+  const int tap = n / u.N, ch = n - tap * u.N;
+  return u.tapoff[tap] + (unsigned)ch;
+}
+ICS_UP8_HD size_t up8_chunk_base_floats(unsigned mbase, const Up8Geom& u) {
+  return (size_t)up8_prow(mbase, u.lgSh, u.P) * (size_t)u.N;
+}
diff --git a/icsg3d_amd/engine.py b/icsg3d_amd/engine.py
--- a/icsg3d_amd/engine.py
+++ b/icsg3d_amd/engine.py
@@ -742,7 +742,9 @@
 
     def kernels(i):
         lines = text.raw[i * cap:(i + 1) * cap].split(b"\0", 1)[0].decode().splitlines()
-        return {k: [ln for ln in lines if ln.startswith("conv_%s:" % k)] for k in ("fwd", "dgrad", "wgrad")}
+        d = {k: [ln for ln in lines if ln.startswith("conv_%s:" % k)] for k in ("fwd", "dgrad", "wgrad")}
+        d["pool"] = [ln for ln in lines if ln.startswith(("pool8:", "pool27:"))]
+        return d
 
     r["kernels"] = [kernels(i) for i in range(R)] if R else kernels(0)
     return r
```

Measured after the change: 1161 (median of 6 runs). 1.2% higher.
